# LittleDang/2DLIW-SLAM

Hardware: AMD Instinct MI355X
Metric: sliding-window solves/sec (30 KF, 2k scan pts) (higher is better)
Workload: dtype f64; 1 GPU; C2 synthetic: 49152 windows/GPU x (n=30 frames, L=2000 laser_factor blocks, 29 IMU + 29 wheel, 1800 ground); step = init-topology LM solve (cap 50 iters) + marginalization per window; windows_per_gpu=49152, frames=30, laser_blocks=2000, parallelism=windows replicated over 1 GPU(s), no data-path collective, distinct_windows_per_gpu=64

## Files before the change

### 2dliw-slam_amd/csrc/k_linearize.hip

```cpp
#include <type_traits>
#include <cstring>
#include "liw_kernels.hpp"

namespace liw {

__device__ __forceinline__ void frame_tf_record(const DevParams& P, const double* pose6, int dir, double* o) {
    V3<LJ> p = cast_v3<LJ>(pose6);
    V3<LJ> th(LJ(pose6[3], dir == 0 ? 1.0 : 0.0), LJ(pose6[4], dir == 1 ? 1.0 : 0.0), LJ(pose6[5], dir == 2 ? 1.0 : 0.0));
    Iso<LJ> Twl = mul(make_tf(p, th), cast_iso<LJ>(P.Ril, P.til));
    const LJ tt[2] = {Twl.t.x, Twl.t.y};
    if (dir == 3) {
        for (int r = 0; r < 2; ++r) { for (int c = 0; c < 3; ++c) o[r * 3 + c] = Twl.R(r, c).v; o[6 + r] = tt[r].v; }
    } else {
        for (int r = 0; r < 2; ++r) { for (int c = 0; c < 3; ++c) o[8 + 6 * dir + r * 3 + c] = Twl.R(r, c).d; o[26 + 2 * dir + r] = tt[r].d; }
    }
}
template <int V, int BIT>
__device__ __forceinline__ void bfly_step(double* v, int lane) {
    if constexpr (V > 1) {
        const bool up = (lane & BIT) != 0;
#pragma unroll
        for (int j = 0; j < V / 2; ++j) {
            const double send = up ? v[j] : v[j + V / 2];
            const double keep = up ? v[j + V / 2] : v[j];
// ... 636 lines not shown
    for (int e = 0; e < PGS; ++e) {
        int r = 0, c = e;
        while (c >= 7 - r) { c -= 7 - r; ++r; }
        t.e[e] = (r << 8) | (c + r);
    }
    return t;
}
__constant__ GroundRcTab c_ground_rc = make_ground_rc();
template <bool COSTCOPY>
__device__ __forceinline__ void ground_frames(const LinArgs& A, const DevParams& P, int wave, double* lds, const int* const act) {
    const int lane = threadIdx.x & 63, sub = lane >> 1, g = lane & 1;
    const int n = A.n;
    const long total = (long)(act ? act[0] : A.B) * n, gf = (long)wave * GROUND_PER_WAVE + sub;
    bool on = gf < total;
    const int wi = on ? (int)(gf / n) : 0;
    const int b = act ? act[1 + wi] : wi;
    if (on && !act) on = window_live(A, b);
    double* Y = lds + sub * 16;
    const size_t fi = on ? (size_t)b * n + (size_t)(gf % n) : 0;
    if (on) {
        const double* s_ = A.x + fi * 15;
        J3 res[2];
        {
            V3<J3> q;
            q.x = seed<3>(s_[3], 0, g == 1); q.y = seed<3>(s_[4], 1, g == 1); q.z = seed<3>(s_[5], 2, g == 1);
            const M3<J3> R = exp_so3(q);
            const J3 pz = seed<3>(s_[2], 2, g == 0);
            res[0] = (R(2, 0) * P.tiw[0] + R(2, 1) * P.tiw[1] + R(2, 2) * P.tiw[2] + pz) * P.ground_p_info;
            const J3 zx = R(0, 0) * P.Riw[2] + R(0, 1) * P.Riw[5] + R(0, 2) * P.Riw[8];
            const J3 zy = R(1, 0) * P.Riw[2] + R(1, 1) * P.Riw[5] + R(1, 2) * P.Riw[8];
            res[1] = dasin(dsqrt(zy * zy + zx * zx)) * P.ground_q_info;
        }
#pragma unroll
        for (int e = 0; e < 3; ++e) { Y[3 * g + e] = res[0].d[e]; Y[7 + 3 * g + e] = res[1].d[e]; }
        if (g == 0) { Y[6] = res[0].v; Y[13] = res[1].v; }
        if (g == 0 && A.dbg_ground_res) { A.dbg_ground_res[fi * 2] = res[0].v; A.dbg_ground_res[fi * 2 + 1] = res[1].v; }
        if (A.dbg_ground_jac)
            for (int e = 0; e < 3; ++e) { A.dbg_ground_jac[(fi * 2) * 6 + 3 * g + e] = res[0].d[e]; A.dbg_ground_jac[(fi * 2 + 1) * 6 + 3 * g + e] = res[1].d[e]; }
    }
    int* meta = reinterpret_cast<int*>(lds + GROUND_PER_WAVE * 16);
    if (g == 0) { meta[sub] = on ? (A.lm ? (A.candidate ? 1 - A.lm[b].cur : A.lm[b].cur) : 0) : -1; meta[32 + sub] = (int)fi; meta[64 + sub] = (int)cs_index(n, b, CS_GROUND, (int)(gf % n)); }
    lds_sync();
    {
        const long gf0 = (long)wave * GROUND_PER_WAVE;
        const int nfr = (int)min((long)GROUND_PER_WAVE, total - gf0);
        const double mult = (double)n;
        constexpr int LPF = PGS / 2;
        const int j = lane / LPF, pr = lane - j * LPF;
        const bool all_on = __builtin_amdgcn_ballot_w64(lane < nfr && meta[lane & 31] < 0) == 0;
        if (j < 4) {
            const int rc0 = c_ground_rc.e[2 * pr], rc1 = c_ground_rc.e[2 * pr + 1];
            const int r0 = rc0 >> 8, c0 = rc0 & 255, r1 = rc1 >> 8, c1 = rc1 & 255;
            auto frame = [&](int q) {
                const double* Yq = lds + q * 16;
                double2 v;
                v.x = mult * __builtin_fma(Yq[7 + r0], Yq[7 + c0], Yq[r0] * Yq[c0]);
                v.y = mult * __builtin_fma(Yq[7 + r1], Yq[7 + c1], Yq[r1] * Yq[c1]);
                return v;
            };
            auto put = [&](int sel, int fq, const double2& v) { *reinterpret_cast<double2*>(&(sel ? A.PG[1] : A.PG[0])[(size_t)fq * PGS + 2 * pr]) = v; };
            int q = j;
            if (all_on)
                for (; q + 4 < nfr; q += 8) {
                    const int sa = meta[q], fa = meta[32 + q], sb = meta[q + 4], fb = meta[36 + q];
                    const double2 va = frame(q), vb = frame(q + 4);
                    put(sa, fa, va); put(sb, fb, vb);
                }
            for (; q < nfr; q += 4) {
                const int sel = meta[q], fq = meta[32 + q];
                const double2 v = frame(q);
                if (sel >= 0) put(sel, fq, v);
            }
        }
        if (COSTCOPY && A.CS[0] && lane < nfr && meta[lane & 31] >= 0) {
            const double* Yq = lds + lane * 16;
            (meta[lane] ? A.CS[1] : A.CS[0])[meta[64 + lane]] = mult * __builtin_fma(Yq[13], Yq[13], Yq[6] * Yq[6]);
        }
    }
}

constexpr int WG_PER_WAVE = 31, WG_REC = 68;
constexpr int WG_LDS = WG_PER_WAVE * WG_REC + 96;
__device__ __forceinline__ LJN<4> ext4(const J3& a) { LJN<4> r; r.v = a.v; r.d[0] = a.d[0]; r.d[1] = a.d[1]; r.d[2] = a.d[2]; r.d[3] = 0.0; return r; }
template <bool COSTCOPY>
__device__ __forceinline__ void wheel_ground2_blocks(const LinArgs& A, const DevParams& P, int wave, double* lds, const int* const act) {
    typedef LJN<4> J4;
    typedef LJN<6> J6;
    const int lane = threadIdx.x & 63, blk = lane >> 1, f = lane & 1;
    const int n = A.n, nb = n - 1;
    const long total = (long)(act ? act[0] : A.B) * nb, gb = (long)wave * A.small_per_wave + blk;
    bool on = blk < A.small_per_wave && blk < WG_PER_WAVE && gb < total;
    const int wi = on ? (int)(gb / nb) : 0, k = on ? (int)(gb % nb) : 0;
    const int b = act ? act[1 + wi] : wi;
    if (on && !act) on = window_live(A, b);
    double* Y = lds + (blk < WG_PER_WAVE ? blk : 0) * WG_REC;
    const size_t fk = on ? (size_t)b * nb + k : 0, fi0 = on ? (size_t)b * n + k : 0;
    if (on) {
        const double* si_ = A.x + fi0 * 15;
        const double* sj_ = si_ + 15;
        const double* T12 = A.wheel_T + fk * 12;
        const double* sq9 = A.wheel_sqrtP + fk * 9;
        const V3<double> thi = cast_v3<double>(si_ + 3), thj = cast_v3<double>(sj_ + 3);
        V3<J3> arg;
        arg.x = seed<3>(f ? thj.x : thi.x, 0, true); arg.y = seed<3>(f ? thj.y : thi.y, 1, true); arg.z = seed<3>(f ? thj.z : thi.z, 2, true);
        const M3<J3> Md = exp_so3(arg);
        M3<double> Ri, Rj;
        {
            const int l0 = lane - f;
#pragma unroll
            for (int q = 0; q < 9; ++q) {
                const double mv = Md.m[q].v;
                Ri.m[q] = __shfl(mv, l0, 64);
                Rj.m[q] = __shfl(mv, l0 + 1, 64);
            }
        }
        {
            const double pz = f ? sj_[2] : si_[2];
            const J3 r0 = (Md(2, 0) * P.tiw[0] + Md(2, 1) * P.tiw[1] + Md(2, 2) * P.tiw[2] + J3(pz)) * P.ground_p_info;
            const J4 zx = ext4(Md(0, 0)) * P.Riw[2] + ext4(Md(0, 1)) * P.Riw[5] + ext4(Md(0, 2)) * P.Riw[8];
            const J4 zy = ext4(Md(1, 0)) * P.Riw[2] + ext4(Md(1, 1)) * P.Riw[5] + ext4(Md(1, 2)) * P.Riw[8];
            const J4 r1 = dasin(dsqrt(zy * zy + zx * zx)) * P.ground_q_info;
            double* Yg = Y + (f ? 39 : 53);
            Yg[0] = 0.0; Yg[1] = 0.0; Yg[2] = P.ground_p_info;
#pragma unroll
            for (int e = 0; e < 3; ++e) { Yg[3 + e] = r0.d[e]; Yg[7 + e] = r1.d[3]; Yg[10 + e] = r1.d[e]; }
            Yg[6] = r0.v; Yg[13] = r1.v;
            const size_t fi = fi0 + f;
            if ((f || k == 0) && A.dbg_ground_res) { A.dbg_ground_res[fi * 2] = r0.v; A.dbg_ground_res[fi * 2 + 1] = r1.v; }
            if ((f || k == 0) && A.dbg_ground_jac)
                for (int e = 0; e < 6; ++e) { A.dbg_ground_jac[(fi * 2) * 6 + e] = Yg[e]; A.dbg_ground_jac[(fi * 2 + 1) * 6 + e] = Yg[7 + e]; }
        }
        __builtin_amdgcn_sched_barrier(0);
        const M3<double> Riw = cast_m3<double>(P.Riw);
        const V3<double> tiw(P.tiw[0], P.tiw[1], P.tiw[2]);
        const M3<double> Rwi = mul(Ri, Riw);
        const M3<double> Am = transpose(Rwi);
        const M3<double> RjRiw = mul(Rj, Riw);
        const V3<double> Rjt = mul(Rj, tiw);
        const V3<double> w(Rjt.x + sj_[0] - si_[0], Rjt.y + sj_[1] - si_[1], Rjt.z + sj_[2] - si_[2]);
        const M3<double> Rrel = mul(Am, RjRiw);
        const V3<double> trel = mul(Am, w) - mulT(Riw, tiw);
        M3<J4> E;
        V3<J6> p;
#pragma unroll
        for (int q = 0; q < 9; ++q) E.m[q] = J4(Rrel.m[q]);
        p.x = J6(trel.x); p.y = J6(trel.y); p.z = J6(trel.z);
        p.x.d[3] = 1.0; p.y.d[4] = 1.0; p.z.d[5] = 1.0;
        {
            const M3<double> RiwT = transpose(Riw);
            M3<double> Lm, Rm;
#pragma unroll
            for (int q = 0; q < 9; ++q) { Lm.m[q] = f == 0 ? RiwT.m[q] : Am.m[q]; Rm.m[q] = f == 0 ? RjRiw.m[q] : Riw.m[q]; }
            const V3<double> wv(f == 0 ? w.x : tiw.x, f == 0 ? w.y : tiw.y, f == 0 ? w.z : tiw.z);
#pragma unroll
            for (int e = 0; e < 3; ++e) {
                M3<double> X;
#pragma unroll
                for (int r = 0; r < 3; ++r)
#pragma unroll
                    for (int c = 0; c < 3; ++c) X(r, c) = f == 0 ? Md(c, r).d[e] : Md(r, c).d[e];
                const M3<double> LX = mul(Lm, X);
                const M3<double> dR = mul(LX, Rm);
                const V3<double> dt = mul(LX, wv);
#pragma unroll
                for (int q = 0; q < 9; ++q) E.m[q].d[e] = dR.m[q];
                p.x.d[e] = dt.x; p.y.d[e] = dt.y; p.z.d[e] = dt.z;
            }
        }
        __builtin_amdgcn_sched_barrier(0);
        const V3<J4> q = log_SO3(E);
        const V3<double> oq = log_SO3(cast_m3<double>(T12));
        const double opx = T12[9], opy = T12[10];
        const double o_len = sqrt(opx * opx + opy * opy);
        const J6 len = dsqrt(p.x * p.x + p.y * p.y);
        J6 res0, res1, angle(0.0);
        if (o_len > 0.0001 && len.v > 0.0001) {
            const double odx = opx / o_len, ody = opy / o_len;
            const J6 dx = p.x / len, dy = p.y / len;
            const J6 cz = dy * odx - dx * ody;
            angle = dasin(dsqrt(cz * cz));
        } else {
            angle = len;
        }
        if (len.v < 0.0001 || o_len < 0.0001) res0 = len * sq9[0];
        else res0 = (J6(o_len) - len) * sq9[0];
        res1 = angle * sq9[4];
        const J4 nq = norm(q);
        const double noq = sqrt(oq.x * oq.x + oq.y * oq.y + oq.z * oq.z);
        J4 res2;
        if (nq.v < 0.001 || noq < 0.001) res2 = nq * sq9[8];
        else res2 = (J4(noq) - nq) * sq9[8];
#pragma unroll
        for (int e = 0; e < 3; ++e) {
            const int col = f ? 9 + e : 3 + e;
            Y[col] = res0.d[e]; Y[13 + col] = res1.d[e]; Y[26 + col] = res2.d[e];
        }
        if (f == 0) {
            const double Dp[3][3] = {{res0.d[3], res0.d[4], res0.d[5]}, {res1.d[3], res1.d[4], res1.d[5]}, {res2.d[3], res2.d[3], res2.d[3]}};
#pragma unroll
            for (int r = 0; r < 3; ++r) {
#pragma unroll
                for (int c = 0; c < 3; ++c) {
                    const double v = Dp[r][0] * Rwi.m[c * 3] + Dp[r][1] * Rwi.m[c * 3 + 1] + Dp[r][2] * Rwi.m[c * 3 + 2];
                    Y[r * 13 + 6 + c] = v;
                    Y[r * 13 + c] = -v;
                }
            }
            Y[12] = res0.v; Y[25] = res1.v; Y[38] = res2.v;
        }
    }
    lds_sync();
    if (on && f == 0 && A.dbg_wheel_res)
        for (int r = 0; r < 3; ++r) A.dbg_wheel_res[fk * 3 + r] = Y[r * 13 + 12];
    if (on && A.dbg_wheel_jac)
        for (int e = f; e < 36; e += 2) A.dbg_wheel_jac[fk * 36 + e] = Y[(e / 12) * 13 + e % 12];
    int* meta = reinterpret_cast<int*>(lds + WG_PER_WAVE * WG_REC);
    if (f == 0 && blk < WG_PER_WAVE) {
        meta[blk] = on ? (A.lm ? (A.candidate ? 1 - A.lm[b].cur : A.lm[b].cur) : 0) : -1;
        meta[32 + blk] = (int)fk;
        meta[64 + blk] = (int)cs_index(n, b, CS_WHEEL, k);
        meta[96 + blk] = (int)fi0;
        meta[128 + blk] = (int)cs_index(n, b, CS_GROUND, k);
        meta[160 + blk] = k;
    }
    lds_sync();
    const long gb0 = (long)wave * A.small_per_wave;
    const int nblk = (int)min((long)min(A.small_per_wave, WG_PER_WAVE), total - gb0);
    const int ml = lane < WG_PER_WAVE ? lane : 0;
    const int selv = meta[ml], fkv = meta[32 + ml], csv = meta[64 + ml], fiv = meta[96 + ml], cgv = meta[128 + ml], kv = meta[160 + ml];
    const bool all_on = __builtin_amdgcn_ballot_w64(lane < nblk && selv < 0) == 0;
    if (lane < PWS / 2) {
        const int rc0 = c_wheel_rc.e[2 * lane], rc1 = c_wheel_rc.e[2 * lane + 1];
        const int r0 = rc0 >> 8, c0 = rc0 & 255;
        const int r1 = rc1 >= 0 ? rc1 >> 8 : 0, c1 = rc1 >= 0 ? rc1 & 255 : 0;
        auto block = [&](int q) {
            const double* Yq = lds + q * WG_REC;
            double2 v;
            v.x = __builtin_fma(Yq[26 + r0], Yq[26 + c0], __builtin_fma(Yq[r0], Yq[c0], Yq[13 + r0] * Yq[13 + c0]));
            const double w1 = __builtin_fma(Yq[26 + r1], Yq[26 + c1], __builtin_fma(Yq[r1], Yq[c1], Yq[13 + r1] * Yq[13 + c1]));
            v.y = rc1 >= 0 ? w1 : 0.0;
            return v;
        };
        auto put = [&](int q, const double2& v) {
            const int sel = __builtin_amdgcn_readlane(selv, q);
            *reinterpret_cast<double2*>(&(sel ? A.PW[1] : A.PW[0])[(size_t)__builtin_amdgcn_readlane(fkv, q) * PWS + 2 * lane]) = v;
        };
        int q = 0;
        if (all_on)
            for (; q + 3 <= nblk; q += 3) {
                const double2 va = block(q), vb = block(q + 1), vc = block(q + 2);
                put(q, va); put(q + 1, vb); put(q + 2, vc);
            }
        for (; q < nblk; ++q) {
            const double2 v = block(q);
            if (__builtin_amdgcn_readlane(selv, q) >= 0) put(q, v);
        }
    }
    {
        const double mult = (double)n;
        constexpr int LPF = PGS / 2;
        const int j = lane / LPF, pr = lane - j * LPF;
        const bool any_k0 = __builtin_amdgcn_ballot_w64(lane < nblk && kv == 0) != 0;
        if (j < 4) {
            const int rc0 = c_ground_rc.e[2 * pr], rc1 = c_ground_rc.e[2 * pr + 1];
            const int r0 = rc0 >> 8, c0 = rc0 & 255, r1 = rc1 >> 8, c1 = rc1 & 255;
            for (int pass = 0; pass < (any_k0 ? 2 : 1); ++pass) {
                const int yo = pass ? 53 : 39;
                for (int q = j; q < nblk; q += 4) {
                    const int sel = meta[q], fq = meta[96 + q] + (pass ? 0 : 1), kq = meta[160 + q];
                    const double* Yq = lds + q * WG_REC + yo;
                    double2 v;
                    v.x = mult * __builtin_fma(Yq[7 + r0], Yq[7 + c0], Yq[r0] * Yq[c0]);
                    v.y = mult * __builtin_fma(Yq[7 + r1], Yq[7 + c1], Yq[r1] * Yq[c1]);
                    if (sel >= 0 && (pass == 0 || kq == 0))
                        *reinterpret_cast<double2*>(&(sel ? A.PG[1] : A.PG[0])[(size_t)fq * PGS + 2 * pr]) = v;
                }
            }
        }
        if (COSTCOPY && A.CS[0] && lane < nblk && selv >= 0) {
            const double* Yq = lds + lane * WG_REC;
            double* CSb = selv ? A.CS[1] : A.CS[0];
            CSb[csv] = __builtin_fma(Yq[38], Yq[38], __builtin_fma(Yq[12], Yq[12], Yq[25] * Yq[25]));
            CSb[cgv + 1] = mult * __builtin_fma(Yq[39 + 13], Yq[39 + 13], Yq[39 + 6] * Yq[39 + 6]);
            if (kv == 0) CSb[cgv] = mult * __builtin_fma(Yq[53 + 13], Yq[53 + 13], Yq[53 + 6] * Yq[53 + 6]);
        }
        (void)fiv;
    }
}

__host__ __device__ inline int imu_wave_count(int B, int n, int per_wave) { return n > 1 ? (int)(((long)B * (n - 1) + per_wave - 1) / per_wave) : 0; }
__host__ __device__ inline int wheel_wave_count(int B, int n, int per_wave) { return imu_wave_count(B, n, per_wave); }
__host__ __device__ inline int ground_wave_count(int B, int n) { return (int)(((long)B * n + GROUND_PER_WAVE - 1) / GROUND_PER_WAVE); }
template <int ND, bool COSTCOPY>
__device__ __forceinline__ void small_role(const LinArgs& A, const DevParams& P, int vblock, double* lds, const int* const act) {
    const int nw = wheel_wave_count(A.B, A.n, A.small_per_wave);
    if (vblock < nw) wheel_blocks<ND, COSTCOPY>(A, P, vblock, lds, act);
    else ground_frames<COSTCOPY>(A, P, vblock - nw, lds, act);
}
constexpr int SMALL_LDS = WHEEL_PER_WAVE * 64 + 32 + 16 + 64;
__global__ __launch_bounds__(64, 2) void k_lin_imu(LinArgs A, DevParams P) {
    __shared__ double lds[IMU_PER_WAVE * IMU_REC];
    const int* const act = usable_active_list(A.active, A.B);
    if (A.imu_pk && *A.imu_pk_bad == 0) imu_blocks<3, true>(A, P, (int)blockIdx.x, lds, act);
    else imu_blocks<3>(A, P, (int)blockIdx.x, lds, act);
}
__global__ __launch_bounds__(64, 2) void k_lin_imu_chain(LinArgs A, DevParams P) {
    __shared__ __attribute__((aligned(16))) double lds[IMU_PER_WAVE * IMU_REC + IMU_STAGE + IMU_SBUF];
    const int* const act = usable_active_list(A.active, A.B);
    if (A.imu_pk && *A.imu_pk_bad == 0) imu_blocks<3, true, true>(A, P, (int)blockIdx.x, lds, act);
    else imu_blocks<3, false, true>(A, P, (int)blockIdx.x, lds, act);
}
__global__ __launch_bounds__(64, 2) void k_lin_imu_chain_multi(LinArgs A, DevParams P) {
    __shared__ __attribute__((aligned(16))) double lds[IMU_PER_WAVE * IMU_REC + IMU_STAGE + IMU_SBUF];
    const int* const act = usable_active_list(A.active, A.B);
    if (A.imu_pk && *A.imu_pk_bad == 0) imu_blocks<3, true, true, true>(A, P, (int)blockIdx.x, lds, act);
    else imu_blocks<3, false, true, true>(A, P, (int)blockIdx.x, lds, act);
}
__global__ void k_imu_pack(long blocks, const double* X, const double* J, const double* S, const double* Dt, double* pk, int* bad) {
    const long t = (long)blockIdx.x * blockDim.x + threadIdx.x;
    if (t >= blocks * 256) return;
    const long fk = t >> 8;
    const int e = (int)(t & 255);
    if (e < IMU_PK) {
        double v = 0.0;
        if (e < 15) v = X[fk * 15 + e];
        else if (e == IPK_DT) v = Dt[fk];
        else if (e < IPK_S) { const int q = e - IPK_J; v = J[fk * 225 + (q / 6) * 15 + 9 + q % 6]; }
        else if (e < IPK_S + 120) {
            int r = 0, q = e - IPK_S;
            while (q >= 15 - r) { q -= 15 - r; ++r; }
            v = S[fk * 225 + r * 15 + r + q];
        }
        pk[fk * IMU_PK + e] = v;
    }
    if (e < 225 && e % 15 < e / 15 && S[fk * 225 + e] != 0.0) atomicOr(bad, 1);
}
__global__ void k_laser_z_scan(long Ltot, const double* pts, int* flag) {
    const long t = (long)blockIdx.x * blockDim.x + threadIdx.x;
    bool nz = false;
    for (long j = t; j < Ltot; j += (long)gridDim.x * blockDim.x)
        nz = nz || pts[2 * Ltot + j] != 0.0 || pts[5 * Ltot + j] != 0.0 || pts[8 * Ltot + j] != 0.0 || pts[11 * Ltot + j] != 0.0;
    if (__any(nz) && (threadIdx.x & 63) == 0) atomicOr(flag, 1);
}
void launch_laser_z_scan(long Ltot, const double* laser_pts, int* flag, hipStream_t s) {
    (void)hipMemsetAsync(flag, 0, sizeof(int), s);
    if (Ltot <= 0) return;
    const long blocks = (Ltot + 1023) / 1024;
    hipLaunchKernelGGL(k_laser_z_scan, dim3((unsigned)(blocks < 4096 ? blocks : 4096)), dim3(256), 0, s, Ltot, laser_pts, flag);
}
void launch_imu_pack(int B, int n, const double* imu_X, const double* imu_J, const double* imu_sqrtP, const double* imu_Dt, double* pk, int* bad, hipStream_t s) {
    (void)hipMemsetAsync(bad, 0, sizeof(int), s);
    const long blocks = (long)B * (n - 1);
    if (blocks <= 0) return;
    hipLaunchKernelGGL(k_imu_pack, dim3((unsigned)blocks), dim3(256), 0, s, blocks, imu_X, imu_J, imu_sqrtP, imu_Dt, pk, bad);
}
constexpr int SMALL_OCC = 2;
__global__ __launch_bounds__(64, SMALL_OCC) void k_lin_small(LinArgs A, DevParams P) {
    __shared__ double lds[WG_LDS > SMALL_LDS ? WG_LDS : SMALL_LDS];
    static_assert(sizeof(double) * (WG_LDS > SMALL_LDS ? WG_LDS : SMALL_LDS) * 4 * SMALL_OCC <= 160 * 1024, "LDS of the waves of a CU");
    const int* const act = usable_active_list(A.active, A.B);
    if (A.n > 1) wheel_ground2_blocks<true>(A, P, (int)blockIdx.x, lds, act);
    else ground_frames<true>(A, P, (int)blockIdx.x, lds, act);
}
__global__ void k_lm_reset(int B, LmState* lm, int max_iters) {
    const int b = blockIdx.x * blockDim.x + threadIdx.x;
    if (b < B) lm_reset(lm[b], max_iters);
}
template <bool BOTH>
__global__ __launch_bounds__(64, 2) void k_lin_all(LinArgs A, DevParams P, int G, int n_laser, int n_imu, int n_roles) {
    __shared__ double lds[IMU_PER_WAVE * IMU_REC];
    const int v = (int)blockIdx.x;
    if (v >= n_roles) {
        for (int b = threadIdx.x; b < A.B; b += 64) lm_reset(A.reset_lm[b], A.reset_iters);
        return;
    }
#ifdef LIW_CLK
    if ((threadIdx.x & 63) == 0 && v < 40) g_clk_lin[400 + 2 * v] = clock64();
#endif
    if (v < n_laser) laser_wave_local<BOTH>(A, P, G, v);
    else if (A.small_nd == 1) {
        if (v < n_laser + n_imu) imu_blocks<1>(A, P, v - n_laser, lds, nullptr); else small_role<1, false>(A, P, v - n_laser - n_imu, lds, nullptr);
    } else {
        if (v < n_laser + n_imu) imu_blocks<3>(A, P, v - n_laser, lds, nullptr); else small_role<3, false>(A, P, v - n_laser - n_imu, lds, nullptr);
    }
#ifdef LIW_CLK
    asm volatile("s_waitcnt vmcnt(0) lgkmcnt(0)" ::: "memory");
    if ((threadIdx.x & 63) == 0 && v < 40) g_clk_lin[401 + 2 * v] = clock64();
#endif
}

constexpr int COMPACT_MAX = 1 << 20;
__host__ __device__ inline size_t compact_pub_offset(int B) { return (sizeof(int) * ((size_t)B + 3) + 7) & ~(size_t)7; }
__host__ __device__ inline size_t compact_list_bytes(int B) { return compact_pub_offset(B) + 8 * (((size_t)B + 255) / 256); }
__global__ __launch_bounds__(256) void k_compact_active(int B, const LmState* lm, int* active) {
    unsigned long long* pub = reinterpret_cast<unsigned long long*>(reinterpret_cast<char*>(active) + compact_pub_offset(B));
    int* ticket = active + B + 1;
    int* status = active + B + 2;
    __shared__ int wcnt[4];
    __shared__ int part[4];
    const int t = threadIdx.x, lane = t & 63, wv = t >> 6, blk = (int)blockIdx.x, nblk = (int)gridDim.x;
    const int b0 = blk * 256 + t;
    const bool live = b0 < B && !lm[b0].done;
    const unsigned long long m = __ballot(live);
    const int before = __popcll(m & ((1ull << lane) - 1ull));
    if (lane == 0) wcnt[wv] = __popcll(m);
    __syncthreads();
    const int bc = wcnt[0] + wcnt[1] + wcnt[2] + wcnt[3];
    if (t == 0) __hip_atomic_store(pub + blk, ((unsigned long long)bc << 1) | 1ull, __ATOMIC_RELEASE, __HIP_MEMORY_SCOPE_AGENT);
    int sum = 0;
    for (int j = t; j < blk; j += 256) {
        unsigned long long v = 0;
        for (long polls = 0; polls < (1l << 24); ++polls) {
            v = __hip_atomic_load(pub + j, __ATOMIC_ACQUIRE, __HIP_MEMORY_SCOPE_AGENT);
            if (v & 1ull) break;
            __builtin_amdgcn_s_sleep(2);
        }
        if (!(v & 1ull)) atomicOr(status, 2);
        sum += (int)(v >> 1);
    }
    for (int o = 32; o > 0; o >>= 1) sum += __shfl_xor(sum, o, 64);
    if (lane == 0) part[wv] = sum;
    __syncthreads();
    const int offset = part[0] + part[1] + part[2] + part[3];
    int wbase = 0;
    for (int q = 0; q < wv; ++q) wbase += wcnt[q];
    if (live) active[1 + offset + wbase + before] = b0;
    if (blk == nblk - 1 && t == 0) { active[0] = offset + bc; atomicOr(status, 1); }
    __syncthreads();
    if (t == 0 && __hip_atomic_fetch_add(ticket, 1, __ATOMIC_ACQ_REL, __HIP_MEMORY_SCOPE_AGENT) == nblk - 1) {
        for (int j = 0; j < nblk; ++j) __hip_atomic_store(pub + j, 0ull, __ATOMIC_RELAXED, __HIP_MEMORY_SCOPE_AGENT);
        __hip_atomic_store(ticket, 0, __ATOMIC_RELEASE, __HIP_MEMORY_SCOPE_AGENT);
    }
}

__global__ void k_group_offsets(int B, int n, const int* laser_off, const int* laser_frame, int* group_off) {
    const int t = blockIdx.x * blockDim.x + threadIdx.x;
    if (t >= B * (n + 1)) return;
    const int b = t / (n + 1), i = t % (n + 1);
    int lo = laser_off[b], hi = laser_off[b + 1];
    while (lo < hi) {
        const int mid = (lo + hi) >> 1;
        if (laser_frame[mid] < i) lo = mid + 1; else hi = mid;
    }
    group_off[t] = lo;
}

size_t compact_list_bytes_host(int B) { return compact_list_bytes(B); }
bool lin_builds_active_list(int B, int eval_small) {
    static const bool no_compact = getenv("LIW_NO_COMPACT") != nullptr;
    return eval_small && B >= 512 && B <= COMPACT_MAX && !no_compact;
}
void launch_linearize(const LinArgs& A_, const DevParams& P, hipStream_t s, const LinFork* fk, bool defer_join) {
    LinArgs A = A_;
    const int n = A.n, B = A.B;
    A.small_nd = 3;
    {
        const long blocks = (long)B * (n > 1 ? n - 1 : 0);
        int pw = WHEEL_PER_WAVE;
        while (pw > 3 && (blocks + pw - 1) / pw < 512) pw = (pw + 1) / 2;
        const bool nd3 = getenv("LIW_SMALL_ND3") != nullptr;
        if (A.eval_small && !nd3 && !A.pi_frame && A.role_mask == 0 && (long)B * n + 2 * blocks + ground_wave_count(B, n) <= 256) { pw = 1; A.small_nd = 1; }
        A.small_per_wave = pw;
        A.imu_per_wave = pw < IMU_PER_WAVE ? pw : IMU_PER_WAVE;
    }
    int G = 1;
    if (A.mode != LIW_MODE_TRACK) while (G < LASER_GMAX && (long)B * ((n + 2 * G - 1) / (2 * G)) >= 4096) G *= 2;
    const int laser_waves = B * ((n + G - 1) / G);
    const int imu_waves = A.eval_small ? imu_wave_count(B, n, A.imu_per_wave) : 0;
    const int small_waves = A.eval_small ? wheel_wave_count(B, n, A.small_per_wave) + ground_wave_count(B, n) : 0;
    const bool have_list = A.lm && A.active && lin_builds_active_list(B, A.eval_small);
    const bool compact = have_list && (A.role_mask == 0 || (A.role_mask & 8));
    if (!have_list) A.active = nullptr;
    if (!A.pi_frame && A.role_mask == 0 && laser_waves + imu_waves + small_waves <= 256) {
        const int roles = laser_waves + imu_waves + small_waves;
        const unsigned tot = (unsigned)(roles + (A.reset_lm ? 1 : 0));
        if (A.mode == LIW_MODE_INIT) hipLaunchKernelGGL(k_lin_all<true>, dim3(tot), dim3(64), 0, s, A, P, G, laser_waves, imu_waves, roles);
        else hipLaunchKernelGGL(k_lin_all<false>, dim3(tot), dim3(64), 0, s, A, P, G, laser_waves, imu_waves, roles);
        return;
    }
    if (A.reset_lm) hipLaunchKernelGGL(k_lm_reset, dim3((B + 63) / 64), dim3(64), 0, s, B, A.reset_lm, A.reset_iters);
    const bool fork = fk && fk->side[0] && A.eval_small;
    if (compact) hipLaunchKernelGGL(k_compact_active, dim3((unsigned)((B + 255) / 256)), dim3(256), 0, s, B, A.lm, A.active);
    if (fork) {
        hipEventRecord(fk->ev_fork, s);
        hipStreamWaitEvent(fk->side[0], fk->ev_fork, 0);
        hipStreamWaitEvent(fk->side[1], fk->ev_fork, 0);
    }
    hipStream_t s_imu = fork ? fk->side[0] : s, s_small = fork ? fk->side[1] : s;
    const int rm = A.role_mask ? A.role_mask : 7;
    auto role_laser = [&]() {
        if (!(rm & 1)) return;
        if (A.laser_pk) launch_lin_laser_slab(A, P, s);
        else if (A.mode == LIW_MODE_INIT) hipLaunchKernelGGL(k_lin_laser<true>, dim3((unsigned)laser_waves), dim3(64), 0, s, A, P, G);
        else hipLaunchKernelGGL(k_lin_laser<false>, dim3((unsigned)laser_waves), dim3(64), 0, s, A, P, G);
    };
    auto role_imu = [&]() {
        const bool no_multi = getenv("LIW_NO_IMU_MULTI") != nullptr;
        if (imu_waves && (rm & 2) && A.pi_frame && imu_chain_windows(n - 1) > 1 && !no_multi) {
            const int wpw = imu_chain_windows(n - 1);
            hipLaunchKernelGGL(k_lin_imu_chain_multi, dim3((unsigned)((B + wpw - 1) / wpw)), dim3(64), 0, s_imu, A, P);
        } else if (imu_waves && (rm & 2) && A.pi_frame) hipLaunchKernelGGL(k_lin_imu_chain, dim3((unsigned)(B * imu_chain_parts(n - 1))), dim3(64), 0, s_imu, A, P);
        else if (imu_waves && (rm & 2)) hipLaunchKernelGGL(k_lin_imu, dim3((unsigned)imu_waves), dim3(64), 0, s_imu, A, P);
    };
    auto role_small = [&]() {
        if (!(small_waves && (rm & 4))) return;
        if (A.small_per_wave == WHEEL_PER_WAVE) A.small_per_wave = WG_PER_WAVE;
        const int waves = n > 1 ? wheel_wave_count(B, n, A.small_per_wave) : ground_wave_count(B, n);
        hipLaunchKernelGGL(k_lin_small, dim3((unsigned)waves), dim3(64), 0, s_small, A, P);
    };
    static const char* order_env = getenv("LIW_LIN_ORDER");
    const char* order = (order_env && strlen(order_env) == 3) ? order_env : "lis";
    for (int k = 0; k < 3; ++k) {
        if (order[k] == 'l') role_laser();
        else if (order[k] == 'i') role_imu();
        else if (order[k] == 's') role_small();
    }
    if (fork) {
        hipEventRecord(fk->ev_join[0], fk->side[0]);
        hipEventRecord(fk->ev_join[1], fk->side[1]);
        if (!defer_join) {
            hipStreamWaitEvent(s, fk->ev_join[0], 0);
            hipStreamWaitEvent(s, fk->ev_join[1], 0);
        }
    }
}
void launch_linearize_join(hipStream_t s, const LinFork* fk) {
    if (!fk || !fk->side[0]) return;
    hipStreamWaitEvent(s, fk->ev_join[0], 0);
    hipStreamWaitEvent(s, fk->ev_join[1], 0);
}

__global__ void k_exchange_pack(int groups, int n, int np, int compact, LaserPackTable tb, const double* PL0, const double* PL1, int candidate, const LmState* lm, double* buf) {
    const int t = blockIdx.x * blockDim.x + threadIdx.x;
    if (t >= groups * np) return;
    const int grp = t / np, p = t % np;
    const bool dead = lm && lm[grp / n].done;
    const int sel = lm ? (candidate ? 1 - lm[grp / n].cur : lm[grp / n].cur) : 0;
    const double* PL = sel ? PL1 : PL0;
    double v;
    if (compact) v = PL[(size_t)grp * LPC + p];
    else { v = PL[(size_t)grp * LP + tb.slot[p]]; v = tb.neg[p] ? -v : v; }
    buf[t] = dead ? 0.0 : v;
}
template <bool BOTH>
__global__ void k_exchange_unpack(int groups, int n, int np, int compact, int world, size_t stride, const double* buf, double* PL0, double* PL1, double* CS0, double* CS1, int candidate, const LmState* lm, int sysload) {
    const int t = blockIdx.x * blockDim.x + threadIdx.x;
    const int lps = laser_stride(compact);
    if (t >= groups * lps) return;
    const int grp = t / lps, s = t % lps;
    const int sel = lm ? (candidate ? 1 - lm[grp / n].cur : lm[grp / n].cur) : 0;
    double* PL = sel ? PL1 : PL0;
    const int code = compact ? (s < np ? s : -1) : laser_slot_code<BOTH>(s);
    double v = 0.0;
    if (code >= 0) {
        const double* src = buf + (size_t)grp * np + (code & 63);
        for (int r = 0; r < world; ++r)
            v += sysload ? __hip_atomic_load(src + (size_t)r * stride, __ATOMIC_RELAXED, __HIP_MEMORY_SCOPE_SYSTEM) : src[(size_t)r * stride];
        if (code & 64) v = -v;
    }
    PL[t] = v;
    if (s == (compact ? np - 1 : 120) && CS0) (sel ? CS1 : CS0)[cs_index(n, grp / n, CS_LASER, grp % n)] = v;
}
template <bool BOTH>
__global__ void k_laser_expand(int groups, int compact, const double* PL, double* out) {
    const size_t t = (size_t)blockIdx.x * blockDim.x + threadIdx.x;
    if (t >= (size_t)groups * LP) return;
    out[t] = laser_slot<BOTH>(PL + (t / LP) * laser_stride(compact), (int)(t % LP), compact);
}
void launch_laser_expand(int B, int n, bool both, int compact, const double* PL, double* out, hipStream_t s) {
    const int groups = B * n;
    const unsigned blocks = (unsigned)(((size_t)groups * LP + 255) / 256);
    if (both) hipLaunchKernelGGL(k_laser_expand<true>, dim3(blocks), dim3(256), 0, s, groups, compact, PL, out);
    else hipLaunchKernelGGL(k_laser_expand<false>, dim3(blocks), dim3(256), 0, s, groups, compact, PL, out);
}
__global__ void k_count_active(int B, const LmState* lm, double* out) {
    __shared__ int cnt;
    if (threadIdx.x == 0) cnt = 0;
    __syncthreads();
    int c = 0;
    for (int b = threadIdx.x; b < B; b += blockDim.x) c += lm[b].done ? 0 : 1;
    atomicAdd(&cnt, c);
    __syncthreads();
    if (threadIdx.x == 0) out[0] = (double)cnt;
}
void launch_exchange_pack(int B, int n, bool both, int compact, const double* PL0, const double* PL1, int candidate, const LmState* lm, double* buf, hipStream_t s) {
    const int np = both ? 45 : 21, groups = B * n;
    LaserPackTable tb{};
    for (int p = 0; p < np; ++p) tb.slot[p] = -1;
    for (int sl = 0; sl < LP; ++sl) {
        const int code = both ? laser_slot_code<true>(sl) : laser_slot_code<false>(sl);
// ... 52 lines not shown
```

### 2dliw-slam_amd/csrc/k_lm.hip

```cpp
#include "liw_kernels.hpp"
#include "k_lm_common.hpp"

namespace liw {

typedef double d4 __attribute__((ext_vector_type(4)));
#ifdef LIW_CLK
__device__ long long g_clk[8192];
__device__ long long g_span[3 * 16384];
#ifndef LIW_CLK_IT
#define LIW_CLK_IT 3
#endif
#define STAMP(id) do { if (b == 0 && lane == 0 && iteration_dbg == LIW_CLK_IT) g_clk[(id)] = clock64(); } while (0)
#define STAMPE(id) do { if (b == 0 && lane == 0 && iteration == LIW_CLK_IT) g_clk[(id)] = clock64(); } while (0)
#define STAMPM(id) do { if (b == 0 && lane == 0) g_clk[(id)] = clock64(); } while (0)
#define JSTAMP(id) do { if (t == 0 && blockIdx.x == 0 && sweep == 1 && rnd == 3) g_clk[(id)] = clock64(); } while (0)
#define JSTAMPV(id, v) do { double w_ = (v); asm volatile("" : "+v"(w_)); if (t == 0 && blockIdx.x == 0 && sweep == 1 && rnd == 3) g_clk[(id)] = clock64(); } while (0)
#define SPAN(k) do { if (lane == 0 && iteration_dbg == LIW_CLK_IT && b < 16384) { g_span[3 * b + (k)] = clock64(); \
                     if ((k) == 0) g_span[3 * b + 2] = __builtin_amdgcn_s_getreg((4 << 0) | (0 << 6) | (31 << 11)); } } while (0)
#else
#define STAMP(id) do { } while (0)
#define STAMPE(id) do { } while (0)
#define STAMPM(id) do { } while (0)
#define JSTAMP(id) do { } while (0)
#define JSTAMPV(id, v) do { } while (0)
#define SPAN(k) do { } while (0)
#endif


struct AsmCtx {
    int n, mode, fast, b, buf;
    int pif;
    int plc;
    const double* PL; const double* PI; const double* PW; const double* PG;
    const double* x;
    const double* pJ; const double* pX; bool prior_on;
};
__device__ __forceinline__ AsmCtx asm_ctx(const WsView& w, int n, int mode, int fast, int b, const double* prior_J, const double* prior_X, bool prior_on) {
    AsmCtx c;
    c.pif = w.pi_frame; c.plc = w.pl_compact; c.n = n; c.mode = mode; c.fast = fast; c.b = b;
    c.pJ = prior_J + (size_t)b * 225; c.pX = prior_X + (size_t)b * 15; c.prior_on = prior_on;
    return c;
}
__device__ __forceinline__ void bind(AsmCtx& c, const WsView& w, int buf, const double* x) {
    c.buf = buf; c.PL = w.PL[buf]; c.PI = w.PI[buf]; c.PW = w.PW[buf]; c.PG = w.PG[buf]; c.x = x;
}

__device__ __forceinline__ void copy_states(double* dst, const double* src, int n, int lane) {
    for (int e = lane; e < n * 15; e += 64) dst[e] = src[e];
}
__device__ __forceinline__ double free_norm(const double* x, int mode, int fast, int n, int lane) {
    double s = 0.0;
    for (int e = lane; e < n * 15; e += 64) if (!var_is_const(mode, fast, n, e / 15, e % 15)) s += x[e] * x[e];
    return sqrt(wave_sum(s));
}
__device__ __forceinline__ void history_put(const StepArgs& a, int rec, int b, const double* x, int lane) {
    if (a.w.history && rec < a.w.history_records)
        for (int e = lane; e < a.n * 15; e += 64) a.w.history[((size_t)rec * a.B + b) * a.n * 15 + e] = x[e];
}
__device__ __forceinline__ void lm_store_exit(LmState& st, int term, double radius, double dec, double x_cost, double x_norm, int reuse, int cur) {
    st.done = 1; st.termination = term; st.radius = radius; st.decrease_factor = dec; st.x_cost = x_cost; st.x_norm = x_norm;
    st.reuse_diagonal = reuse; st.cur = cur; st.have_candidate = 0;
}

__device__ __forceinline__ double prior_r(const AsmCtx& c, int k) {
    const double* xs = c.x + (size_t)(c.n - 2) * 15;
    double s = 0.0;
    for (int j = 0; j < 15; ++j) s += c.pJ[k * 15 + j] * (xs[j] - c.pX[j]);
    return s;
}

__device__ __forceinline__ double pl_slot(const AsmCtx& c, const double* rec, int s) { return laser_slot(rec, s, c.plc, c.mode == LIW_MODE_INIT); }

struct FrameExtra { double sc_i, sc_m, dg_i, x_i; };

constexpr int MS = 41;
template <int LAYOUT> struct Tiles {
    double* D; double* O; double* R; double* g;
    __device__ __forceinline__ double& d(int r, int c) const { return LAYOUT ? D[r * MS + c] : D[r * 16 + c]; }
    __device__ __forceinline__ double& o(int r, int c) const { return LAYOUT ? D[c * MS + 16 + r] : O[r * 16 + c]; }
    __device__ __forceinline__ double& rr(int r, int c) const { return LAYOUT ? D[c * MS + 32 + r] : R[r * 16 + c]; }
    __device__ __forceinline__ double& gg(int r) const { return LAYOUT ? D[r * MS + 40] : g[r]; }
};

struct AsmRegs {
    double v5[4], v6[4], v7[4];
    double t1, t2, t3, t4, t8, t9, t10;
    double g1, g2, g3, g4, g5, g6;
    double xq, sc_i, sc_m, dg_i;
    double e1[2], e2;
};
struct PriorRegs { double pj[4], pdx; };
__device__ __forceinline__ PriorRegs prior_issue(const AsmCtx& c, int lane) {
    PriorRegs P;
#pragma unroll
    for (int q = 0; q < 4; ++q) {
        const int e = lane + 64 * q, r = e >> 4, cc = e & 15;
        P.pj[q] = (r < 15 && cc < 15) ? c.pJ[r * 15 + cc] : 0.0;
    }
    const int v = lane < 15 ? lane : 0;
    P.pdx = c.x[(size_t)(c.n - 2) * 15 + v] - c.pX[v];
    return P;
}
constexpr int ASM_TMP = 16;

__device__ __forceinline__ AsmRegs asm_issue(const AsmCtx& c, int i, const double* scl, const double* dgl, int lane = threadIdx.x & 63, int dir = -1) {
    const int n = c.n;
    const bool up = dir > 0;
    const int LPS = laser_stride(c.plc);
    const double* PLb = c.PL + (size_t)c.b * n * LPS;
    const bool pif = c.pif != 0;
    const bool hasm = i >= 1, hasp = i <= n - 2;
    const double* PIb = c.PI + (size_t)c.b * (pif ? (size_t)n * PIFS : (size_t)(n - 1) * PIS);
    const double* PWb = c.PW + (size_t)c.b * (n - 1) * PWS;
    const double* PGb = c.PG + (size_t)c.b * n * PGS;
    const double* PIm = pif ? PIb + (size_t)i * PIFS : PIb + (size_t)(hasm ? i - 1 : 0) * PIS;
    const double* PIp = pif ? PIb + (size_t)(hasp ? i + 1 : i) * PIFS : PIb + (size_t)(hasp ? i : 0) * PIS;
    const int oJJ = pif ? PIF_D : PI_JJ, oIJ = pif ? PIF_IJ : PI_IJ;
    const double* PWm = PWb + (size_t)(hasm ? i - 1 : 0) * PWS;
    const double* PWp = PWb + (size_t)(hasp ? i : 0) * PWS;
    const double* PLi = PLb + (size_t)i * LPS;
    const double* PL1 = PLb + (size_t)(n > 1 ? 1 : 0) * LPS;
    const double* PGi = PGb + (size_t)i * PGS;
    AsmRegs R;
#pragma unroll
    for (int q = 0; q < 4; ++q) {
        const int e = lane + 64 * q, r = e >> 4, cc = e & 15;
        const bool valid = r < 15 && cc < 15;
        const int rs = valid ? r : 0, cs = valid ? cc : 0;
        const int tq = pi_tri(rs, cs);
        R.v5[q] = PIm[(unsigned)(oJJ + tq)];
        R.v6[q] = pif ? 0.0 : PIp[(unsigned)(PI_II + tq)];
        R.v7[q] = up ? PIp[(unsigned)(oIJ + cs * 15 + rs)] : PIm[(unsigned)(oIJ + rs * 15 + cs)];
    }
    {
        const bool pl = lane < 36;
        const int r = pl ? lane / 6 : 0, cc = pl ? lane % 6 : 0;
        R.t1 = pl_slot(c, PLi, 36 + r * 6 + cc);
        R.t2 = PWm[(unsigned)PW_JJ(r, cc)];
        R.t3 = PWp[(unsigned)PW_II(r, cc)];
        R.t4 = PGi[(unsigned)PG_H(r, cc)];
        R.t8 = up ? PWp[(unsigned)PW_IJ(cc, r)] : PWm[(unsigned)PW_IJ(r, cc)];
        R.e2 = up ? PWm[(unsigned)PW_IJ(r, cc)] : 0.0;
        R.t9 = pl_slot(c, PL1, 72 + r * 6 + cc);
        R.t10 = pl_slot(c, PLi, 72 + r * 6 + cc);
    }
    {
        const int r = lane < 15 ? lane : 0, r6 = r < 6 ? r : 0;
        R.g1 = pl_slot(c, PLi, 114 + r6);
        R.g2 = PWm[(unsigned)PW_G(6 + r6)];
        R.g3 = PWp[(unsigned)PW_G(r6)];
        R.g4 = PGi[(unsigned)PG_G(r6)];
        R.g5 = PIm[(unsigned)((pif ? PIF_GJ : PI_G + 15) + r)];
        R.g6 = pif ? PIm[(unsigned)(PIF_GI + r)] : PIp[(unsigned)(PI_G + r)];
    }
    const int nbf = up ? (hasp ? i + 1 : i) : (hasm ? i - 1 : i);
    {
        int idx = i * 15 + (lane < 15 ? lane : 0);
        if (lane >= 16 && lane < 19) idx = nbf * 15 + 3 + (lane - 16);
        if (lane >= 20 && lane < 23) idx = 3 + (lane - 20);
        R.xq = c.x[(unsigned)idx];
        const int v = lane < 15 ? lane : 0;
        R.sc_i = scl ? scl[(unsigned)(i * 15 + v)] : 1.0;
        R.sc_m = scl ? scl[(unsigned)(nbf * 15 + v)] : 1.0;
        R.dg_i = dgl ? dgl[(unsigned)(i * 15 + v)] : 0.0;
    }
#pragma unroll
    for (int q = 0; q < 2; ++q) {
        const int e = lane + 64 * q;
        R.e1[q] = up ? PIm[(unsigned)(oIJ + (e < 90 ? e : 0))] : 0.0;
    }
    return R;
}

__device__ __forceinline__ d4 xty16(const double* X, const double* Y);
template <int LAYOUT>
__device__ void asm_commit(const AsmCtx& c, int i, const AsmRegs& R, const Tiles<LAYOUT>& T_, double* tmp, FrameExtra* ex = nullptr,
                           int lane = threadIdx.x & 63, int dir = -1, const PriorRegs* pr = nullptr) {
    const int n = c.n;
    const int LPS = laser_stride(c.plc);
    const double* PLb = c.PL + (size_t)c.b * n * LPS;
    const bool hasm = i >= 1, hasp = i <= n - 2;
    const bool up = dir > 0, hasnb = up ? hasp : hasm;
    const int nbf = up ? (hasp ? i + 1 : i) : (hasm ? i - 1 : i);
    const bool arrow1 = up && i == 1;
    const bool prior_here = c.prior_on && i == n - 2;
    d4 jtj = {0.0, 0.0, 0.0, 0.0};
    double gprior = 0.0;
    if (prior_here) {
        double* Jt = T_.D;
        double* dxp = LAYOUT ? T_.D + 256 : T_.O;
        const PriorRegs P_ = pr ? *pr : prior_issue(c, lane);
#pragma unroll
        for (int q = 0; q < 4; ++q) Jt[lane + 64 * q] = P_.pj[q];
        if (lane < 16) dxp[lane] = lane < 15 ? P_.pdx : 0.0;
        lds_sync();
        if (lane < 15) {
            double sp = 0.0;
#pragma unroll
            for (int j = 0; j < 15; ++j) sp += Jt[lane * 16 + j] * dxp[j];
            tmp[lane] = sp;
        }
        jtj = xty16(Jt, Jt);
        lds_sync();
        if (lane < 15) {
#pragma unroll
            for (int k = 0; k < 15; ++k) gprior += Jt[k * 16 + lane] * tmp[k];
        }
        lds_sync();
    }
    double dI[4], oI[4];
#pragma unroll
    for (int q = 0; q < 4; ++q) {
        const int e = lane + 64 * q, r = e >> 4, cc = e & 15;
        const bool valid = r < 15 && cc < 15;
        dI[q] = ((valid && (c.pif ? n > 1 : hasm)) ? R.v5[q] : 0.0) + ((valid && hasp && !c.pif) ? R.v6[q] : 0.0);
        oI[q] = (valid && hasnb) ? R.v7[q] : 0.0;
    }
    double dP = 0.0, oP = 0.0, rP = 0.0;
    {
        const bool pl = lane < 36;
        const int r = pl ? lane / 6 : 0, cc = pl ? lane % 6 : 0;
        dP = R.t1 + (hasm ? R.t2 : 0.0) + (hasp ? R.t3 : 0.0) + R.t4;
        if (i == 0 && c.mode == LIW_MODE_INIT) {
            double s0 = 0.0, s1 = 0.0, s2 = 0.0, s3 = 0.0;
            int j = 0;
            for (; j + 4 <= n; j += 4) {
                s0 += pl_slot(c, PLb + (size_t)j * LPS, r * 6 + cc); s1 += pl_slot(c, PLb + (size_t)(j + 1) * LPS, r * 6 + cc);
                s2 += pl_slot(c, PLb + (size_t)(j + 2) * LPS, r * 6 + cc); s3 += pl_slot(c, PLb + (size_t)(j + 3) * LPS, r * 6 + cc);
            }
            for (; j < n; ++j) s0 += pl_slot(c, PLb + (size_t)j * LPS, r * 6 + cc);
            dP += (s0 + s1) + (s2 + s3);
        }
        oP = hasnb ? R.t8 + ((!up && i == 1) ? R.t9 : 0.0) : 0.0;
        rP = (i >= 2 || arrow1) ? R.t10 + (arrow1 ? R.e2 : 0.0) : 0.0;
        if (!pl) { dP = 0.0; oP = 0.0; rP = 0.0; }
    }
    double gg = 0.0;
    {
        const int r = lane < 15 ? lane : 0;
        if (r < 6) {
            gg = R.g1 + (hasm ? R.g2 : 0.0) + (hasp ? R.g3 : 0.0) + R.g4;
            if (i == 0 && c.mode == LIW_MODE_INIT) {
                double s0 = 0.0, s1 = 0.0, s2 = 0.0, s3 = 0.0;
                int j = 0;
                for (; j + 4 <= n; j += 4) {
                    s0 += pl_slot(c, PLb + (size_t)j * LPS, 108 + r); s1 += pl_slot(c, PLb + (size_t)(j + 1) * LPS, 108 + r);
                    s2 += pl_slot(c, PLb + (size_t)(j + 2) * LPS, 108 + r); s3 += pl_slot(c, PLb + (size_t)(j + 3) * LPS, 108 + r);
                }
                for (; j < n; ++j) s0 += pl_slot(c, PLb + (size_t)j * LPS, 108 + r);
                gg += (s0 + s1) + (s2 + s3);
            }
        }
        gg += (hasm ? R.g5 : 0.0) + (hasp ? R.g6 : 0.0);
    }
    const double xq = R.xq;
    if (ex) { ex->sc_i = R.sc_i; ex->sc_m = R.sc_m; ex->dg_i = R.dg_i; ex->x_i = xq; }
#pragma unroll
    for (int q = 0; q < 4; ++q) {
        const int e = lane + 64 * q;
        const int r = e >> 4, cc = e & 15;
        const bool valid = r < 15 && cc < 15;
        double d = dI[q];
        if (prior_here && valid) d += jtj[q];
        if (LAYOUT == 0) { T_.D[e] = valid ? d : 0.0; T_.O[e] = valid ? oI[q] : 0.0; T_.R[e] = 0.0; }
        else if (valid) { T_.d(r, cc) = d; T_.o(r, cc) = oI[q]; if (r < 6) T_.rr(r, cc) = 0.0; }
    }
    if (lane < 16) {
        double g = lane < 15 ? gg : 0.0;
        if (prior_here && lane < 15) g += gprior;
        if (LAYOUT == 0) T_.g[lane] = g; else if (lane < 15) T_.gg(lane) = g;
    }
    lds_sync();
    if (lane < 36) {
        const int r = lane / 6, cc = lane % 6;
        T_.d(r, cc) += dP; T_.o(r, cc) += oP; T_.rr(r, cc) = rP;
    }
    lds_sync();
    if (arrow1) {
#pragma unroll
        for (int q = 0; q < 2; ++q) {
            const int e = lane + 64 * q;
            if (e < 90) T_.rr(e / 15, e % 15) += R.e1[q];
        }
        lds_sync();
    }
    if (c.mode == LIW_MODE_MARG) return;
    double Pi[9], Pm[9], P0[9];
    const double qa0 = rdlane(xq, 3), qa1 = rdlane(xq, 4), qa2 = rdlane(xq, 5);
    const double qb0 = rdlane(xq, 16), qb1 = rdlane(xq, 17), qb2 = rdlane(xq, 18);
    const double qc0 = rdlane(xq, 20), qc1 = rdlane(xq, 21), qc2 = rdlane(xq, 22);
    const double pi2 = kPi * kPi;
    bool li = qa0 * qa0 + qa1 * qa1 + qa2 * qa2 > pi2;
    bool lm = hasnb && qb0 * qb0 + qb1 * qb1 + qb2 * qb2 > pi2;
    bool l0 = (i >= 2 || arrow1) && qc0 * qc0 + qc1 * qc1 + qc2 * qc2 > pi2;
    if (li || lm || l0) {
        li = so3_plus_jac(c.x + (size_t)i * 15 + 3, Pi);
        lm = hasnb && so3_plus_jac(c.x + (size_t)nbf * 15 + 3, Pm);
        l0 = (i >= 2 || arrow1) && so3_plus_jac(c.x + 3, P0);
        if (lane == 0) {
            auto at = [&](int kind, int r, int cc) -> double& { return kind == 0 ? T_.d(r, cc) : (kind == 1 ? T_.o(r, cc) : T_.rr(r, cc)); };
            auto right = [&](int kind, int nrows, const double* P) {
                for (int r = 0; r < nrows; ++r) {
                    double t[3];
                    for (int k = 0; k < 3; ++k) t[k] = at(kind, r, 3) * P[k] + at(kind, r, 4) * P[3 + k] + at(kind, r, 5) * P[6 + k];
                    for (int k = 0; k < 3; ++k) at(kind, r, 3 + k) = t[k];
                }
            };
            auto left = [&](int kind, const double* P) {
                for (int cc = 0; cc < 15; ++cc) {
                    double t[3];
                    for (int k = 0; k < 3; ++k) t[k] = P[k] * at(kind, 3, cc) + P[3 + k] * at(kind, 4, cc) + P[6 + k] * at(kind, 5, cc);
                    for (int k = 0; k < 3; ++k) at(kind, 3 + k, cc) = t[k];
                }
            };
            if (li) {
                right(0, 15, Pi); left(0, Pi); right(1, 15, Pi); right(2, 6, Pi);
                double t[3];
                for (int k = 0; k < 3; ++k) t[k] = Pi[k] * T_.gg(3) + Pi[3 + k] * T_.gg(4) + Pi[6 + k] * T_.gg(5);
                for (int k = 0; k < 3; ++k) T_.gg(3 + k) = t[k];
            }
            if (lm) left(1, Pm);
            if (l0) left(2, P0);
        }
        lds_sync();
    }
    if (c.mode == LIW_MODE_TRACK) {
        for (int e = lane; e < 256; e += 64) {
            const int r = e >> 4, cc = e & 15;
            if (r < 15 && cc < 15) {
                const bool cr = var_is_const(c.mode, c.fast, n, i, r), ccn = var_is_const(c.mode, c.fast, n, i, cc);
                if (cr || ccn) T_.d(r, cc) = 0.0;
                if ((hasnb && var_is_const(c.mode, c.fast, n, nbf, r)) || ccn) T_.o(r, cc) = 0.0;
                if (arrow1 && r < 6 && (var_is_const(c.mode, c.fast, n, 0, r) || ccn)) T_.rr(r, cc) = 0.0;
            }
        }
        if (lane < 15 && var_is_const(c.mode, c.fast, n, i, lane)) T_.gg(lane) = 0.0;
        lds_sync();
    }
}

template <int LAYOUT>
__device__ void assemble_frame(const AsmCtx& c, int i, const Tiles<LAYOUT>& T_, double* tmp,
                               const double* scl = nullptr, const double* dgl = nullptr, FrameExtra* ex = nullptr) {
    const AsmRegs R = asm_issue(c, i, scl, dgl);
    __builtin_amdgcn_sched_barrier(0);
    asm_commit<LAYOUT>(c, i, R, T_, tmp, ex);
}

__device__ double window_cost(const AsmCtx& c, double* gchk = nullptr) {
    const int lane = threadIdx.x & 63;
    const int n = c.n;
    const int LPS = laser_stride(c.plc);
    const double* PLb = c.PL + (size_t)c.b * n * LPS;
    const bool pif = c.pif != 0;
    const double* PIb = c.PI + (size_t)c.b * (pif ? (size_t)n * PIFS : (size_t)(n - 1) * PIS);
    const double* PWb = c.PW + (size_t)c.b * (n - 1) * PWS;
    const double* PGb = c.PG + (size_t)c.b * n * PGS;
    const bool track = c.mode == LIW_MODE_TRACK;
    double s = 0.0, gs = 0.0;
    for (int i = lane; i < n; i += 64) {
        const bool gon = !(track && i < n - 1);
        if (gon) s += pl_slot(c, PLb + (size_t)i * LPS, 120);
        if (gon) s += PGb[(size_t)i * PGS + PG_C];
        if (gchk) {
            if (gon) {
#pragma unroll
                for (int k = 0; k < 12; ++k) gs += pl_slot(c, PLb + (size_t)i * LPS, 108 + k);
            }
            if (gon) {
#pragma unroll
                for (int k = 0; k < 6; ++k) gs += PGb[(size_t)i * PGS + PG_G(k)];
            }
        }
    }
    for (int k = lane; k < n - 1; k += 64) {
        s += pif ? PIb[(size_t)(k + 1) * PIFS + PIF_C] : PIb[(size_t)k * PIS + PI_C];
        const bool won = !(track && k < n - 2);
        if (won) s += PWb[(size_t)k * PWS + PW_C];
        if (gchk) {
#pragma unroll
            for (int e = 0; e < 30; ++e)
                gs += pif ? (e < 15 ? PIb[(size_t)k * PIFS + PIF_GI + e] : PIb[(size_t)(k + 1) * PIFS + PIF_GJ + e - 15]) : PIb[(size_t)k * PIS + PI_G + e];
            if (won) {
#pragma unroll
                for (int e = 0; e < 12; ++e) gs += PWb[(size_t)k * PWS + PW_G(e)];
            }
        }
    }
    if (c.prior_on && lane < 15) { const double r = prior_r(c, lane); s += r * r; }
    if (gchk) *gchk = wave_sum(gs);
    return 0.5 * wave_sum(s);
}

__device__ __forceinline__ d4 xty16(const double* X, const double* Y) {
    const int lane = threadIdx.x & 63;
    d4 acc = {0.0, 0.0, 0.0, 0.0};
#pragma unroll
    for (int c = 0; c < 4; ++c) {
        const int k = (lane >> 4) + 4 * c;
        acc = __builtin_amdgcn_mfma_f64_16x16x4f64(X[k * 16 + (lane & 15)], Y[k * 16 + (lane & 15)], acc, 0, 0, 0);
    }
    return acc;
}

template <int XS, int YS>
__device__ __forceinline__ d4 xty15(const double* X, const double* Y, const double* Z) {
    const int lane = threadIdx.x & 63, m = lane & 15;
    d4 acc = {0.0, 0.0, 0.0, 0.0};
#pragma unroll
    for (int c = 0; c < 4; ++c) {
        const int k = (lane >> 4) + 4 * c;
        const double* xr = X + k * XS;
        const double* yr = Y + k * YS;
        if (c == 3) { const bool z = (lane >> 4) == 3; xr = z ? Z : xr; yr = z ? Z : yr; }
        acc = __builtin_amdgcn_mfma_f64_16x16x4f64(xr[m], yr[m], acc, 0, 0, 0);
    }
    return acc;
}

struct LdsTiles {
    double D[256], O[256], R[256], W[256], Wa[256], CD[256], CR[256];
    double g[16], Cg[16], y0[16], yprev[16], tmp[ASM_TMP], D0acc[36], g0acc[8], sci[16], scm[16], sc0[16], dgi[16];
};
struct LdsStep {
    double M[720], C[15 * MS], Z[16];
    double tmp[ASM_TMP], D0acc[36], g0acc[8];
};
constexpr int LW = 0, LLI = 240, LWA = 480;
struct LdsDense2 {
    LdsStep S;
    double D1[256], O1[256], R1[256], D0[256], O0[256], R0[256], g1[16], g0[16];
};
__device__ __forceinline__ LdsStep& step_lds(LdsStep& T) { return T; }
__device__ __forceinline__ LdsStep& step_lds(LdsDense2& T) { return T.S; }

template <int NP = 15>
__device__ __forceinline__ bool fused_chol_solve(double (&a)[15]) {
    bool ok = true;
#pragma unroll
    for (int k = 0; k < NP; ++k) {
        const double piv = rdlane(a[k], k);
        if (k == NP - 1 && (!(piv > 0.0) || !isfinite(piv))) ok = false;
        const double inv = fast_rsqrt(piv);
        const double wk = a[k] * inv;
        a[k] = wk;
#pragma unroll
        for (int r = k + 1; r < 15; ++r) a[r] -= rdlane(wk, r) * wk;
    }
    return ok;
}

__device__ __forceinline__ bool fused_chol_solve30(double (&a)[30], unsigned inert) {
    bool ok = true;
#pragma unroll
    for (int k = 0; k < 30; ++k) {
        if (k < 15 && ((inert >> k) & 1u)) continue;
        const double piv = rdlane(a[k], k);
        if (k == 29 && (!(piv > 0.0) || !isfinite(piv))) ok = false;
        const double inv = fast_rsqrt(piv);
        const double wk = a[k] * inv;
        a[k] = wk;
#pragma unroll
        for (int r = k + 1; r < 30; ++r) a[r] -= rdlane(wk, r) * wk;
    }
    return ok;
}

template <bool WAVE_ONLY = false>
__device__ double frame_diag(const AsmCtx& c, int i, LdsStep& T) {
    const int lane = threadIdx.x & 63, n = c.n;
    double Pq[9];
    if (so3_plus_jac(c.x + (size_t)i * 15 + 3, Pq)) {
        assemble_frame<1>(c, i, Tiles<1>{T.M, nullptr, nullptr, nullptr}, T.tmp);
        const double d = lane < 15 ? T.M[lane * MS + lane] : 0.0;
        lds_sync();
        return d;
    }
    if (lane >= 15) return 0.0;
    const int r = lane;
    const int LPS = laser_stride(c.plc);
    const double* PLb = c.PL + (size_t)c.b * n * LPS;
    const double* PIb = c.PI + (size_t)c.b * (c.pif ? (size_t)n * PIFS : (size_t)(n - 1) * PIS);
    const double* PWb = c.PW + (size_t)c.b * (n - 1) * PWS;
    const double* PGb = c.PG + (size_t)c.b * n * PGS;
    double d = 0.0;
    if (r < 6) {
        d += pl_slot(c, PLb + (size_t)i * LPS, 36 + r * 7);
        if (i == 0) for (int j = 0; j < n; ++j) d += pl_slot(c, PLb + (size_t)j * LPS, r * 7);
        if (i >= 1) d += PWb[(size_t)(i - 1) * PWS + PW_JJ(r, r)];
        if (i <= n - 2) d += PWb[(size_t)i * PWS + PW_II(r, r)];
        d += PGb[(size_t)i * PGS + PG_H(r, r)];
    }
    if (c.pif) { if (n > 1) d += PIb[(size_t)i * PIFS + PIF_D + pi_tri(r, r)]; }
    else {
        if (i >= 1) d += PIb[(size_t)(i - 1) * PIS + PI_JJ + pi_tri(r, r)];
        if (i <= n - 2) d += PIb[(size_t)i * PIS + PI_II + pi_tri(r, r)];
    }
    if (c.prior_on && i == n - 2) { double s = 0.0; for (int k = 0; k < 15; ++k) s += c.pJ[k * 15 + r] * c.pJ[k * 15 + r]; d += s; }
    return d;
}

struct BsRow { double row[22], gsv, xold, scv, dgv; };
__device__ __forceinline__ BsRow bs_fetch(const double* sws, const double* xw, const double* scl, const double* dgl, int i, int lane) {
    static_assert(REC_LD % 2 == 0 && SOLVE_WS % 2 == 0, "16-byte aligned record rows");
    const double* f = sws + (size_t)i * SOLVE_WS;
    const int r = lane < 15 ? lane : 0;
    const double2* f2 = reinterpret_cast<const double2*>(f + r * REC_LD);
    BsRow R;
#pragma unroll
    for (int k = 0; k < 11; ++k) { const double2 v = f2[k]; R.row[2 * k] = v.x; R.row[2 * k + 1] = v.y; }
    R.gsv = f[REC_GS + r]; R.xold = xw[(size_t)i * 15 + r]; R.scv = scl[i * 15 + r]; R.dgv = dgl[i * 15 + r];
    return R;
}
__device__ __forceinline__ void bs_emit(const StepArgs& a, int i, int lane, double t, const BsRow& R, double damp, double* xc, double& sn2, double& ytg, double& dsum) {
    const bool cst = lane < 15 && var_is_const(a.mode, a.fast_mode, a.n, i, lane);
    const double del = (lane < 15 && !cst) ? -t * R.scv : 0.0;
    const double qv[3] = {rdlane(R.xold, 3), rdlane(R.xold, 4), rdlane(R.xold, 5)};
    double dq[3] = {rdlane(del, 3), rdlane(del, 4), rdlane(del, 5)}, qn[3];
    so3_plus(qv, dq, qn);
    if (lane < 15) {
        double xnew = R.xold + del;
        if (lane >= 3 && lane < 6) xnew = var_is_const(a.mode, a.fast_mode, a.n, i, 3) ? R.xold : qn[lane - 3];
        xc[(size_t)i * 15 + lane] = xnew;
        if (!cst) {
            sn2 += (R.xold - xnew) * (R.xold - xnew);
            ytg += t * R.gsv;
            dsum += damp * t * t;
        }
    }
}

template <bool THROUGHPUT, bool DENSE2 = false, class LDS = LdsStep>
__device__ __forceinline__ void lm_step_body(const StepArgs& a, const int b, LDS& TL) {
    constexpr bool LIW_PF1 = !THROUGHPUT, LIW_PF2 = true;
    LdsStep& T = step_lds(TL);
    const int lane = threadIdx.x & 63;
    LmState& st = a.w.lm[b];
    if constexpr (DENSE2) {
        double pf_sink = 0.0;
        int done0 = st.done;
        const int n2 = a.n;
        const bool pr = a.mode == LIW_MODE_TRACK && !a.fast_mode;
        double v[14];
#pragma unroll
        for (int k = 0; k < 2; ++k) {
            v[4 * k + 0] = touch_lines(a.w.PL[k] + (size_t)b * n2 * laser_stride(a.w.pl_compact), sizeof(double) * n2 * laser_stride(a.w.pl_compact));
            v[4 * k + 1] = touch_lines(a.w.PI[k] + (size_t)b * (n2 - 1) * PIS, sizeof(double) * (n2 - 1) * PIS);
            v[4 * k + 2] = touch_lines(a.w.PW[k] + (size_t)b * (n2 - 1) * PWS, sizeof(double) * (n2 - 1) * PWS);
            v[4 * k + 3] = touch_lines(a.w.PG[k] + (size_t)b * n2 * PGS, sizeof(double) * n2 * PGS);
        }
        v[8] = touch_lines(a.x + (size_t)b * n2 * 15, sizeof(double) * n2 * 15);
        v[9] = touch_lines(a.w.x_cand + (size_t)b * n2 * 15, sizeof(double) * n2 * 15);
        v[10] = touch_lines(st.scale, sizeof(double) * n2 * 15);
        v[11] = touch_lines(st.diagonal, sizeof(double) * n2 * 15);
        {
            const double* const xb = a.x + (size_t)b * n2 * 15;
            const double* const PJ = a.prior_J; const double* const PX = a.prior_X;
            const bool pj = pr && PJ != nullptr, px = pr && PX != nullptr;
            const size_t qj = (size_t)(PJ + (size_t)b * 225), qx = (size_t)(PX + (size_t)b * 15), q0 = (size_t)xb;
            v[12] = touch_lines(reinterpret_cast<const void*>(pj ? qj : q0), pj ? sizeof(double) * 225 : sizeof(double) * 8);
            v[13] = touch_lines(reinterpret_cast<const void*>(px ? qx : q0), px ? sizeof(double) * 15 : sizeof(double) * 8);
        }
#pragma unroll
        for (int k = 0; k < 14; ++k) pf_sink += v[k];
        asm volatile("" : "+v"(pf_sink), "+v"(done0));
        if (done0) return;
    }
    if (st.done) return;
    if (a.only_slow) {
        const int taken = st.pad_;
        wave_mem_sync();
        if (taken) { if (lane == 0) st.pad_ = 0; return; }
    }
    const int n = a.n;
// ... 814 lines not shown
        } else if (a.mode == LIW_MODE_TRACK) {
            if (i == n - 1 && a.has_match[i]) a.match_pose[i * 12 + 6 + k] = a.x[(size_t)i * 15 + k];
        }
    }
    __syncthreads();
    int* hdr = reinterpret_cast<int*>(a.out);
    if (t == 0) { hdr[0] = a.lm[0].done; hdr[1] = a.marg_status ? a.marg_status[0] : 3; hdr[2] = 0; }
    if (t == 1) {
        const LmState& st = a.lm[0];
        liw_summary o;
        o.iterations = st.iteration; o.successful_steps = st.successful; o.termination = st.termination;
        o.initial_cost = st.initial_cost; o.final_cost = st.x_cost;
        *reinterpret_cast<liw_summary*>(a.out + 2) = o;
        a.info[0] = o;
    }
    double* o = a.out + LIW_RESULT_HDR;
    for (int e = t; e < n * 15; e += blockDim.x) o[e] = a.x[e];
    o += n * 15;
    for (int e = t; e < n * 12; e += blockDim.x) o[e] = a.match_pose[e];
    o += n * 12;
    if (a.marg) for (int e = t; e < 276; e += blockDim.x) o[e] = a.marg[e];
    __threadfence_system();
    __syncthreads();
    if (t == 0) { __threadfence_system(); __hip_atomic_store(hdr + 3, a.seq, __ATOMIC_RELEASE, __HIP_MEMORY_SCOPE_SYSTEM); }
}
__global__ void k_pack_result(PackArgs a) { pack_result_body(a); }

__global__ void k_lm_finish(StepArgs a) {
    const int t = blockIdx.x * blockDim.x + threadIdx.x;
    const int n = a.n;
    if (t >= a.B * n * 6) return;
    const int k = t % 6, i = (t / 6) % n, b = t / (6 * n);
    const double* xw = a.x + (size_t)b * n * 15;
    double* mp = a.match_pose + (size_t)b * n * 12;
    if (a.mode == LIW_MODE_INIT) {
        if (a.has_match[b * n + i]) { mp[i * 12 + k] = xw[k]; mp[i * 12 + 6 + k] = xw[(size_t)i * 15 + k]; }
    } else if (a.mode == LIW_MODE_TRACK) {
        if (i == n - 1 && a.has_match[b * n + i]) mp[i * 12 + 6 + k] = xw[(size_t)i * 15 + k];
    }
    if (i == 0 && k == 0) {
        const LmState& st = a.w.lm[b];
        liw_summary& o = a.w.info[b];
        o.iterations = st.iteration; o.successful_steps = st.successful; o.termination = st.termination;
        o.initial_cost = st.initial_cost; o.final_cost = st.x_cost;
    }
}

__global__ __launch_bounds__(64) void k_export_dense(ExportArgs a) {
    __shared__ LdsTiles T;
    const int b = blockIdx.x, lane = threadIdx.x & 63, n = a.n, N = 15 * n;
    AsmCtx c = asm_ctx(a.w, n, a.mode, a.fast_mode, b, a.prior_J, a.prior_X,
                       a.has_prior[b] && ((a.mode == LIW_MODE_TRACK && !a.fast_mode) || a.mode == LIW_MODE_MARG));
    bind(c, a.w, 0, a.x + (size_t)b * n * 15);
    c.buf = a.buf;
    double* H = a.H + (size_t)b * N * N;
    double* g = a.g + (size_t)b * N;
    for (size_t e = lane; e < (size_t)N * N; e += 64) H[e] = 0.0;
    __syncthreads();
    const double sgn = a.mode == LIW_MODE_MARG ? -1.0 : 1.0;
    for (int i = 0; i < n; ++i) {
        assemble_frame<0>(c, i, Tiles<0>{T.D, T.O, T.R, T.g}, T.tmp);
        for (int e = lane; e < 256; e += 64) {
            const int r = e >> 4, cc = e & 15;
            if (r < 15 && cc < 15) {
                H[(size_t)(i * 15 + r) * N + i * 15 + cc] = T.D[e];
                if (i >= 1) { H[(size_t)((i - 1) * 15 + r) * N + i * 15 + cc] = T.O[e]; H[(size_t)(i * 15 + cc) * N + (i - 1) * 15 + r] = T.O[e]; }
                if (i >= 2 && r < 6) { H[(size_t)r * N + i * 15 + cc] = T.R[e]; H[(size_t)(i * 15 + cc) * N + r] = T.R[e]; }
            }
        }
        if (lane < 15) g[i * 15 + lane] = sgn * T.g[lane];
        __syncthreads();
    }
    const double cst = window_cost(c);
    if (lane == 0) a.cost[b] = cst;
}

template <class TILES>
__device__ __forceinline__ bool marg_chain(const MargArgs& a, const int b, TILES& T) {
    const int lane = threadIdx.x & 63, n = a.n;
    AsmCtx c = asm_ctx(a.w, n, LIW_MODE_MARG, 0, b, a.prior_J, a.prior_X, a.has_prior[b] != 0);
    const int sel = a.use_cur ? __builtin_amdgcn_readfirstlane(a.w.lm[b].cur) : 0;
    c.buf = sel; c.x = a.x + (size_t)b * n * 15;
    c.PL = sel ? a.w.PL[1] : a.w.PL[0]; c.PI = sel ? a.w.PI[1] : a.w.PI[0]; c.PW = sel ? a.w.PW[1] : a.w.PW[0]; c.PG = sel ? a.w.PG[1] : a.w.PG[0];
    STAMPM(5000);
    for (int e = lane; e < 256; e += 64) { T.CD[e] = 0.0; T.W[e] = 0.0; }
    if (lane < 16) T.Cg[lane] = 0.0;
    lds_sync();
    bool ok = true;
    double* Dc = T.D; double* gc = T.g;
    double* Dn = T.Wa; double* gn = T.y0;
    assemble_frame<0>(c, 0, Tiles<0>{Dc, T.O, T.R, gc}, T.tmp);
    AsmRegs areg = asm_issue(c, n > 1 ? 1 : 0, nullptr, nullptr);
    for (int i = 0; i + 1 < n; ++i) {
        asm_commit<0>(c, i + 1, areg, Tiles<0>{Dn, T.O, T.R, gn}, T.tmp);
        __builtin_amdgcn_sched_barrier(0);
        if (i + 2 < n) areg = asm_issue(c, i + 2, nullptr, nullptr);
        __builtin_amdgcn_sched_barrier(0);
        double col[15];
        {
            const bool ml_ = lane < 15, ol_ = lane >= 16 && lane < 31, gl_ = lane == 40;
            const double* pA = ml_ ? Dc + lane : (ol_ ? T.O + (lane - 16) : (gl_ ? gc : T.R));
            const double* pB = ml_ ? T.CD + lane : (gl_ ? T.Cg : (ol_ ? T.Cg + 15 : T.R));
            const int st = gl_ ? 1 : 16, stB = ol_ ? 0 : st;
#pragma unroll
            for (int r = 0; r < 15; ++r) col[r] = pA[r * st] + pB[r * stB];
        }
        if (!fused_chol_solve(col)) { ok = false; break; }
        if ((lane >= 16 && lane < 31) || lane == 40) {
            double* const wc = T.W + (lane == 40 ? 15 : lane - 16);
#pragma unroll
            for (int r = 0; r < 15; ++r) wc[r * 16] = col[r];
        }
        lds_sync();
        const d4 p1 = xty16(T.W, T.W);
        lds_sync();
#pragma unroll
        for (int r = 0; r < 4; ++r) {
            const int row = (lane >> 4) + 4 * r, colx = lane & 15;
            if (row < 15 && colx < 15) T.CD[row * 16 + colx] = -p1[r];
            if (row < 15 && colx == 15) T.Cg[row] = -p1[r];
        }
        lds_sync();
        double* t1 = Dc; Dc = Dn; Dn = t1;
        double* t2 = gc; gc = gn; gn = t2;
    }
    {
        double dv[4], gv = 0.0;
#pragma unroll
        for (int q = 0; q < 4; ++q) {
            const int e = lane + 64 * q, r = e >> 4, cc = e & 15;
            dv[q] = (r < 15 && cc < 15) ? Dc[e] + T.CD[e] : 0.0;
        }
        if (lane < 15) gv = gc[lane] + T.Cg[lane];
        lds_sync();
#pragma unroll
        for (int q = 0; q < 4; ++q) T.D[lane + 64 * q] = dv[q];
        if (lane < 16) T.g[lane] = lane < 15 ? gv : 0.0;
        lds_sync();
    }
    if (a.status && lane == 0) a.status[b] = ok ? 0 : 1;
    if (!ok) return false;
    if (a.Delta_H) for (int e = lane; e < 225; e += 64) a.Delta_H[(size_t)b * 225 + e] = T.D[(e / 15) * 16 + e % 15];
    if (a.Delta_g && lane < 15) a.Delta_g[(size_t)b * 15 + lane] = -T.g[lane];
    return true;
}

__device__ __forceinline__ void jacobi_rotation(double d, double h, double& cs, double& sn) {
    const double qq = d * d + h * h;
    const double r = qq * fast_rsqrt(qq);
    const double u = fabs(d) + r;
    const double winv = fast_rsqrt(2.0 * r * u);
    cs = u * winv;
    sn = (d >= 0.0 ? h : -h) * winv;
}
template <class TILES>
__device__ __forceinline__ void jacobi15_wave(TILES& T, double* V, double* Am, double* rot) {
    const int lane = threadIdx.x & 63;
    for (int e = lane; e < 256; e += 64) {
        const int r = e >> 4, cc = e & 15;
        Am[e] = (r < 15 && cc < 15) ? 0.5 * (T.D[r * 16 + cc] + T.D[cc * 16 + r]) : 0.0;
        V[e] = r == cc ? 1.0 : 0.0;
    }
    lds_sync();
    for (int sweep = 0; sweep < 60; ++sweep) {
        double off = 0.0, dgn = 0.0;
        for (int e = lane; e < 225; e += 64) {
// ... 410 lines not shown
```

### 2dliw-slam_amd/csrc/k_lm_quad.hip

```cpp
#include <cstddef>
#include <cstdlib>
#include <type_traits>

#include "liw_kernels.hpp"
#include "k_lm_common.hpp"

namespace liw {

template <int B_, int E_, class F> __device__ __forceinline__ void sfor(F&& f) {
    if constexpr (B_ < E_) { f(std::integral_constant<int, B_>{}); sfor<B_ + 1, E_>(f); }
}
#define KI(K) (std::remove_reference_t<decltype(K)>::value)
template <int V> using KC = std::integral_constant<int, V>;
__device__ __forceinline__ double bits_and(double x, unsigned long long m) { return __longlong_as_double((long long)((unsigned long long)__double_as_longlong(x) & m)); }

template <int L> __device__ __forceinline__ double bc(double v) {
    double r;
    asm volatile("v_mov_b64_dpp %0, %1 row_newbcast:%2 row_mask:0xf bank_mask:0xf" : "=v"(r) : "v"(v), "n"(L));
    return r;
}
template <int L> __device__ __forceinline__ void fnma_bc(double& acc, double src, double mul) {
    asm volatile("v_fmac_f64_dpp %0, -%1, %2 row_newbcast:%3 row_mask:0xf bank_mask:0xf" : "+v"(acc) : "v"(src), "v"(mul), "n"(L));
}
template <int L> __device__ __forceinline__ double mul_bc(double src, double mul) {
    double r;
    asm volatile("v_mul_f64_dpp %0, %1, %2 row_newbcast:%3 row_mask:0xf bank_mask:0xf" : "=v"(r) : "v"(src), "v"(mul), "n"(L));
    return r;
}
__device__ __forceinline__ double mul_nop(double x, double y) {
    double r;
    asm volatile("v_mul_f64 %0, %1, %2\n s_nop 1" : "=v"(r) : "v"(x), "v"(y));
    return r;
}
__device__ __forceinline__ void dpp_fence() { asm volatile("s_nop 1"); }

__device__ __forceinline__ double row_max(double v) {
    v = fmax(v, dpp64<0xB1>(v, v)); v = fmax(v, dpp64<0x4E>(v, v)); v = fmax(v, dpp64<0x141>(v, v)); v = fmax(v, dpp64<0x140>(v, v));
    return v;
}

__device__ long long g_qclk[64];
__device__ int g_qclk_on[4];
#define QSTAMP(id) do { if (clk_on && i == clk_frame) { if (lane == 0) g_qclk[(id)] = clock64(); } } while (0)

constexpr int QTR = 4 * 15 * 6;
constexpr int K_A = 0, K_B = 6, K_C = 12, K_HA = 18, K_D = 24, K_CW = 39, K_GSH = 45, K_RL = 46, NRD = 52;
constexpr int QTAB = NRD * 16;
constexpr int QZB = 86;
constexpr int QPAD = 96;
constexpr int QTOT_1 = 4 * (PIFS + LPC + PWS + PGS) + QPAD + QTR + QZB + QTAB;
constexpr int quad_laser_slot(int kind, int r, int j) {
    return kind == 0 ? (j == 15 ? 114 + r : 36 + r * 6 + j) : kind == 1 ? (j == 15 ? 108 + r : r * 6 + j) : 72 + j * 6 + r;
}
template <bool BOTH> constexpr bool quad_sign_rows_ok() {
    for (int jj = 0; jj < 7; ++jj) {
        const int j = jj < 6 ? jj : 15;
        auto sg = [&](int kind, int r) { const int c = laser_slot_code<BOTH>(quad_laser_slot(kind, r, j)); return c >= 0 && (c & 64) != 0; };
        for (int r = 0; r < 6; ++r) {
            if (sg(1, r)) return false;
            if (sg(0, r) != (r < 2 ? sg(0, 0) : (r > 2 && sg(0, 3)))) return false;
            if (j < 6 && sg(2, r) != (r < 2 && sg(2, 0))) return false;
        }
        if (sg(0, 0) != sg(0, 1) || (j < 6 && sg(2, 0) != sg(2, 1))) return false;
    }
    return true;
}
static_assert(quad_sign_rows_ok<true>() && quad_sign_rows_ok<false>(), "sign rows of the laser reads");
template <bool BOTH> constexpr unsigned long long quad_code_pack(int kind, int r) {
    unsigned long long v = 0;
    for (int jj = 0; jj < 7; ++jj) {
        const int c = (kind == 2 && jj == 6) ? -1 : laser_slot_code<BOTH>(quad_laser_slot(kind, r, jj < 6 ? jj : 15));
        v |= (unsigned long long)(c < 0 ? 0xff : c) << (8 * jj);
    }
    return v;
}
template <int KIND, int R> __device__ __forceinline__ int quad_code(bool track, int role) {
    constexpr unsigned long long both = quad_code_pack<true>(KIND, R), one = quad_code_pack<false>(KIND, R);
    const int c = (int)(((track ? one : both) >> (8 * role)) & 0xffull);
    return c == 0xff ? -1 : c;
}
__device__ __forceinline__ double flip_sign(double x, unsigned m) { return __hiloint2double(__double2hiint(x) ^ (int)m, __double2loint(x)); }
constexpr int BSD2 = 3;
constexpr int QTOT_2 = BSD2 * (((4 * REC_GS + 127) / 128) * 128 + 6 * 32);
constexpr int QTOT = QTOT_1 > QTOT_2 ? QTOT_1 : QTOT_2;

template <int R> __device__ __forceinline__ int tri_rc(int j, int cj) {
    constexpr int cR = 14 * R - (R * (R - 1)) / 2;
    return R <= j ? cR + j : cj + R;
}

__global__ __launch_bounds__(64, 1) void k_lm_step_quad(StepArgs a) {
    __shared__ double S[QTOT];
    const int lane = threadIdx.x & 63, j = lane & 15, w = lane >> 4;
    const int n = a.n;
    const bool track = a.mode == LIW_MODE_TRACK;
    const int fast = a.fast_mode;
    auto is_const = [&](int i, int v) { return track && i < n - 1 && (v < 6 || (fast && v >= 9)); };
    int b = (int)blockIdx.x * 4 + w;
    bool act;
    const int* const alist = a.use_active ? usable_active_list(a.w.active, a.B) : nullptr;
    if (alist) {
        act = b < alist[0];
        b = act ? alist[1 + b] : 0;
        if ((unsigned)b >= (unsigned)a.B) { act = false; b = 0; }
    } else {
        act = b < a.B;
        b = act ? b : a.B - 1;
    }
    double* const X = a.x;
    double* const XC = a.w.x_cand;
    double* const LMD = reinterpret_cast<double*>(a.w.lm);
    constexpr unsigned LMS = sizeof(LmState) / 8, LM_SCALE = offsetof(LmState, scale) / 8, LM_DIAG = offsetof(LmState, diagonal) / 8,
                       LM_X0 = offsetof(LmState, x0) / 8;
    const unsigned oX = (unsigned)b * (unsigned)(n * 15), oLM = (unsigned)b * LMS;
    LmState& st = a.w.lm[b];
    act = act && !st.done;
    const int have_cand = st.have_candidate;
    {
        const double sl = quad_slow_lane(X + oX, XC + oX, have_cand, n, j, 16) ? 1.0 : 0.0;
        act = act && !(row_max(sl) > 0.0);
    }
    if (act && j == 0) st.pad_ = 1;
    if (!__any(act)) return;

    int reuse = st.reuse_diagonal, cur = st.cur;
    const int iteration = st.iteration;
    bool proceed = act, last_successful = true;
    const bool fresh = iteration == 0 && !have_cand;
    const bool clk_k = g_qclk_on[0] && (int)blockIdx.x == g_qclk_on[1] && iteration == g_qclk_on[3] && lane == 0;
    if (clk_k) g_qclk[12] = clock64();
    double inv_radius;
    {
        double radius = st.radius, dec = st.decrease_factor, x_cost = st.x_cost, x_norm = st.x_norm;
        const int max_iters = st.max_iters, successful0 = st.successful;
        int successful = successful0;
        const double model0 = st.model_cost_change, cand_step_norm = st.cand_step_norm, initial_cost0 = st.initial_cost;
        double minimum_cost = st.minimum_cost, initial_cost = initial_cost0;
        const int cb = (fresh || !have_cand) ? cur : 1 - cur;
        double cost;
        {
            const double* CSb = (cb ? a.w.CS[1] : a.w.CS[0]) + cs_index(n, b, 0, 0);
            double s = 0.0;
            for (int i = j; i < n; i += 16) {
                s += CSb[CS_LASER * n + i];
                if (!(track && i < n - 1)) s += CSb[CS_GROUND * n + i];
            }
            for (int k = j; k < n - 1; k += 16) {
                s += CSb[CS_IMU * n + k];
                if (!(track && k < n - 2)) s += CSb[CS_WHEEL * n + k];
            }
            if (track && !fast && a.has_prior[b] && j < 15) {
                const double* xs = ((fresh || !have_cand) ? X : XC) + oX + (unsigned)((n - 2) * 15);
                const double* pJ = a.prior_J + (size_t)b * 225 + j * 15;
                const double* pX = a.prior_X + (size_t)b * 15;
                double r = 0.0;
#pragma unroll
                for (int q = 0; q < 15; ++q) r += pJ[q] * (xs[q] - pX[q]);
                s += r * r;
            }
            cost = 0.5 * row_sum(s);
        }
        int term = 0;
        bool accept = false, fail_eval = false;
        if (fresh) {
            x_cost = cost; initial_cost = cost; minimum_cost = cost;
            fail_eval = !isfinite(cost);
        } else if (have_cand) {
            const double cand_cost = isfinite(cost) ? cost : kFailedEvalCost;
            term = lm_candidate_term(cand_step_norm, x_norm, x_cost, cand_cost);
            if (!term) {
                const double rho = (x_cost - cand_cost) / model0;
                accept = lm_accepts(rho);
                if (accept) {
                    cur = cb; x_cost = cand_cost;
                    lm_step_accepted(rho, radius, dec, reuse);
                    successful += 1;
                    if (x_cost < minimum_cost) minimum_cost = x_cost;
                } else {
                    lm_step_rejected(radius, dec, reuse);
                    last_successful = false;
                }
            }
        } else {
            last_successful = false;
        }
        {
            double s2 = 0.0;
            const bool restore = act && fail_eval && !fresh && successful0 > 0;
            const bool hist = act && a.w.history && iteration < a.w.history_records && !fail_eval;
            for (int e0 = j; e0 < n * 15; e0 += 16 * 8) {
                double xv[8];
#pragma unroll
                for (int q = 0; q < 8; ++q) {
                    const int e = e0 + 16 * q;
                    const unsigned ee = (unsigned)(e < n * 15 ? e : j);
                    xv[q] = restore ? LMD[oLM + LM_X0 + ee] : (accept ? XC[oX + ee] : X[oX + ee]);
                }
#pragma unroll
                for (int q = 0; q < 8; ++q) {
                    const int e = e0 + 16 * q;
                    if (e < n * 15) {
                        if (act && (accept || restore)) X[oX + (unsigned)e] = xv[q];
                        if (act && fresh) LMD[oLM + LM_X0 + (unsigned)e] = xv[q];
                        if (!is_const(e / 15, e % 15)) s2 += xv[q] * xv[q];
                        if (hist) a.w.history[((size_t)iteration * a.B + b) * (size_t)(n * 15) + e] = xv[q];
                    }
                }
            }
            s2 = row_sum(s2);
            if (fresh || accept) x_norm = sqrt(s2);
        }
        if (act && (fail_eval || term)) {
            if (j == 0) {
                st.done = 1; st.termination = fail_eval ? 6 : term;
                if (fail_eval) { st.x_cost = fresh ? cost : initial_cost0; st.have_candidate = 0; if (!fresh) st.iteration = iteration - 1; }
                if (fresh) { st.initial_cost = initial_cost; st.minimum_cost = minimum_cost; }
            }
            proceed = false;
        }
        const bool cap = proceed && lm_cap_reached(iteration, max_iters, fresh);
        if (proceed && j == 0) {
            st.radius = radius; st.decrease_factor = dec; st.x_cost = x_cost; st.x_norm = x_norm; st.cur = cur;
            st.successful = successful; st.minimum_cost = minimum_cost;
            if (fresh) st.initial_cost = initial_cost;
            if (cap) { st.done = 1; st.termination = 4; st.reuse_diagonal = reuse; st.have_candidate = 0; }
        }
        if (cap) proceed = false;
        inv_radius = 1.0 / radius;
    }
    if (!__any(proceed)) return;

    const double* const PL0 = a.w.PL[0];
    const double* const PI0 = a.w.PI[0];
    const double* const PW0 = a.w.PW[0];
    const double* const PG0 = a.w.PG[0];
    const unsigned oPL = (unsigned)b * (unsigned)(n * LPC) + (cur ? (unsigned)(a.w.PL[1] - a.w.PL[0]) : 0u);
    const unsigned oPI = (unsigned)b * (unsigned)(n * PIFS) + (cur ? (unsigned)(a.w.PI[1] - a.w.PI[0]) : 0u);
    const unsigned oPW = (unsigned)b * (unsigned)((n - 1) * PWS) + (cur ? (unsigned)(a.w.PW[1] - a.w.PW[0]) : 0u);
    const unsigned oPG = (unsigned)b * (unsigned)(n * PGS) + (cur ? (unsigned)(a.w.PG[1] - a.w.PG[0]) : 0u);
    const unsigned oWS = (unsigned)b * (unsigned)(n * SOLVE_WS);
    double* const WS = a.w.solve_ws;
    const unsigned oSC = oLM + LM_SCALE, oDG = oLM + LM_DIAG;
    const int jc = j < 15 ? j : 0;
    const bool l6 = j < 6, lm = j < 15;

    const bool prior_row = track && !fast && a.has_prior[b] != 0;
    if (__any(proceed && fresh)) {
        double sp = 0.0;
        if (prior_row) for (int k = 0; k < 15; ++k) { const double v = a.prior_J[(size_t)b * 225 + k * 15 + jc]; sp += v * v; }
        const int cbb = track ? laser_slot_code<false>(36 + (l6 ? jc : 0) * 7) : laser_slot_code<true>(36 + (l6 ? jc : 0) * 7);
        const int caa = track ? laser_slot_code<false>((l6 ? jc : 0) * 7) : laser_slot_code<true>((l6 ? jc : 0) * 7);
        for (int i0 = 0; i0 < n; i0 += 4) {
            double vbb[4], vjj[4], vii[4], vg[4], vi[4];
#pragma unroll
            for (int u = 0; u < 4; ++u) {
                const int i = min(i0 + u, n - 1);
                const int j6 = l6 ? jc : 0;
                vbb[u] = PL0[oPL + (unsigned)(i * LPC + (cbb >= 0 ? cbb & 63 : 0))];
                vbb[u] = cbb >= 0 ? vbb[u] : 0.0;
                vjj[u] = n > 1 ? PW0[oPW + (unsigned)(max(i - 1, 0) * PWS + PW_JJ(j6, j6))] : 0.0;
                vii[u] = n > 1 ? PW0[oPW + (unsigned)(min(i, n - 2) * PWS + PW_II(j6, j6))] : 0.0;
                vg[u] = PG0[oPG + (unsigned)(i * PGS + PG_H(j6, j6))];
                vi[u] = PI0[oPI + (unsigned)(i * PIFS + PIF_D + pi_tri(jc, jc))];
            }
#pragma unroll
            for (int u = 0; u < 4; ++u) {
                const int i = i0 + u;
                if (i >= n) break;
                double dd = 0.0;
                if (l6) {
                    dd += vbb[u];
                    if (i == 0) for (int f = 0; f < n; ++f) { const double va = PL0[oPL + (unsigned)(f * LPC + (caa >= 0 ? caa & 63 : 0))]; dd += caa >= 0 ? va : 0.0; }
                    if (i >= 1) dd += vjj[u];
                    if (i <= n - 2) dd += vii[u];
                    dd += vg[u];
                }
                if (n > 1) dd += vi[u];
                if (prior_row && i == n - 2) dd += sp;
                if (proceed && fresh && lm) LMD[oSC + (unsigned)(i * 15 + j)] = is_const(i, j) ? 1.0 : 1.0 / (1.0 + sqrt(dd));
            }
        }
    }
    const double sc0 = l6 ? LMD[oSC + (unsigned)jc] : 0.0;

    constexpr int S_IMU = 0, S_PL = 4 * PIFS, S_PW = S_PL + 4 * LPC, S_PG = S_PW + 4 * PWS, S_TR = S_PG + 4 * PGS + QPAD;
    constexpr int S_ZERO = S_TR + QTR, S_TAB = S_ZERO + QZB;
    static_assert(S_TAB + QTAB <= QTOT && 8 * QTOT < 65536, "LDS layout");
    const unsigned rPI[4] = {(unsigned)__builtin_amdgcn_readlane(oPI, 0), (unsigned)__builtin_amdgcn_readlane(oPI, 16), (unsigned)__builtin_amdgcn_readlane(oPI, 32), (unsigned)__builtin_amdgcn_readlane(oPI, 48)};
    const unsigned rPW[4] = {(unsigned)__builtin_amdgcn_readlane(oPW, 0), (unsigned)__builtin_amdgcn_readlane(oPW, 16), (unsigned)__builtin_amdgcn_readlane(oPW, 32), (unsigned)__builtin_amdgcn_readlane(oPW, 48)};
    const unsigned oPGw = oPG + (unsigned)(PG0 - PW0);
    const unsigned oPLw = oPL + (unsigned)(PL0 - PW0);
    const unsigned rPLw[4] = {(unsigned)__builtin_amdgcn_readlane(oPLw, 0), (unsigned)__builtin_amdgcn_readlane(oPLw, 16), (unsigned)__builtin_amdgcn_readlane(oPLw, 32), (unsigned)__builtin_amdgcn_readlane(oPLw, 48)};
    const unsigned rPGw[4] = {(unsigned)__builtin_amdgcn_readlane(oPGw, 0), (unsigned)__builtin_amdgcn_readlane(oPGw, 16), (unsigned)__builtin_amdgcn_readlane(oPGw, 32), (unsigned)__builtin_amdgcn_readlane(oPGw, 48)};
    typedef __attribute__((address_space(3))) void* lds_t;
    const int j_ = j;
    double scm_n = 1.0, dg_n = 0.0, xq_n = 0.0;
    auto prefetch_regs = [&](int f) {
        const int jq = j_ < 15 ? j_ : 0;
        scm_n = (j_ < 15 && f >= 1) ? LMD[oSC + (unsigned)((f - 1) * 15 + jq)] : 1.0;
        dg_n = LMD[oDG + (unsigned)(f * 15 + jq)];
        xq_n = X[oX + (unsigned)(f * 15 + jq)];
    };
    auto prefetch = [&](int f) {
        asm volatile("s_waitcnt lgkmcnt(0)" ::: "memory");
        const int k = f - 1;
        int lane2 = lane * 2;
        asm volatile("" : "+v"(lane2));
        if (n > 1) {
            sfor<0, 4>([&](auto W) {
                constexpr int ws = KI(W);
                const double* g = PI0 + rPI[ws] + (unsigned)(f * PIFS) + lane2;
                sfor<0, 3>([&](auto Q) { __builtin_amdgcn_global_load_lds(g, (lds_t)(S + S_IMU + ws * PIFS), 16, KI(Q) * 1024, 0); });
            });
        }
        {
            const unsigned fl = (unsigned)(f * LPC), fw = (unsigned)((k >= 0 ? k : 0) * PWS), fg = (unsigned)(f * PGS);
            constexpr int NPC = (4 * (LPC + PWS + PGS) + 127) / 128;
            static_assert(NPC * 128 - 4 * (LPC + PWS + PGS) <= QPAD && LPC % 2 == 0 && PWS % 2 == 0 && PGS % 2 == 0, "stream pieces: pad, 16-byte slots");
            sfor<0, NPC>([&](auto P) {
                constexpr int q0 = KI(P) * 128;
                unsigned off = 0;
                sfor<0, 12>([&](auto G) {
                    constexpr int g = KI(G);
                    constexpr int st = g < 4 ? g * LPC : g < 8 ? 4 * LPC + (g - 4) * PWS : 4 * (LPC + PWS) + (g - 8) * PGS;
                    constexpr int en = g == 11 ? (1 << 20) : st + (g < 4 ? LPC : g < 8 ? PWS : PGS);
                    if constexpr (st < q0 + 128 && en > q0) {
                        const unsigned v = (g < 4 ? rPLw[g & 3] + fl : g < 8 ? rPW[g & 3] + fw : rPGw[g & 3] + fg) + (unsigned)(lane2 - (st - q0));
                        if constexpr (st <= q0) off = v; else off = lane2 >= st - q0 ? v : off;
                    }
                });
                __builtin_amdgcn_global_load_lds(PW0 + off, (lds_t)(S + S_PL + q0), 16, 0, 0);
            });
        }
        asm volatile("" ::: "memory");
        prefetch_regs(f);
    };
    const double* SI = S + S_IMU + w * PIFS;
    unsigned short* const TAB = reinterpret_cast<unsigned short*>(S + S_TAB);
    {
        const int jt = j < 15 ? j : 0, cjt = 14 * jt - (jt * (jt - 1)) / 2, j6t = j < 6 ? j : 0;
        const bool t6 = j < 6, t15 = j == 15, tm = j < 15;
        const int oL = S_PL + w * LPC, oW_ = S_PW + w * PWS, oG = S_PG + w * PGS, oI = S_IMU + w * PIFS;
        auto put = [&](int k, bool on, int idx) { TAB[k * 64 + lane] = (unsigned short)(8 * (on ? idx : S_ZERO)); };
        const int role = t15 ? 6 : j6t;
        auto put_laser = [&](int k, bool on, int code) { put(k, on && code >= 0, oL + (code & 63)); };
        for (int e = lane; e < QZB; e += 64) S[S_ZERO + e] = 0.0;
        sfor<0, 6>([&](auto R) {
            constexpr int r = KI(R);
            put_laser(K_A + r, t6 || t15, quad_code<0, r>(track, role));
            put(K_B + r, t6 || t15, oW_ + (t15 ? PW_G(6 + r) : PW_JJ(r, j6t)));
            put(K_C + r, t6 || t15, oG + (t15 ? PG_G(r) : PG_H(r, j6t)));
            put_laser(K_HA + r, t6 || t15, quad_code<1, r>(track, role));
            put(K_CW + r, t6 || t15, oW_ + (t15 ? PW_G(r) : PW_II(r, j6t)));
            put_laser(K_RL + r, t6, quad_code<2, r>(track, role));
        });
        put(K_GSH, t6, oW_ + PW_G(j6t));
        sfor<0, 15>([&](auto R) {
            constexpr int r = KI(R);
            put(K_D + r, tm, oI + PIF_D + tri_rc<r>(jt, cjt));
        });
    }
    unsigned sgA0, sgA3, sgR0;
    {
        const bool t6 = j < 6, t15 = j == 15;
        const int role = t15 ? 6 : (t6 ? j : 0);
        const int cA0 = quad_code<0, 0>(track, role), cA3 = quad_code<0, 3>(track, role), cR0 = quad_code<2, 0>(track, role);
        sgA0 = ((t6 || t15) && cA0 >= 0 && (cA0 & 64)) ? 0x80000000u : 0u;
        sgA3 = ((t6 || t15) && cA3 >= 0 && (cA3 & 64)) ? 0x80000000u : 0u;
        sgR0 = (t6 && cR0 >= 0 && (cR0 & 64)) ? 0x80000000u : 0u;
    }
    const int lane_tab = lane * 2;
    auto RD = [&](auto K) -> double {
        constexpr int k = KI(K);
        const unsigned off = *reinterpret_cast<const unsigned short*>(reinterpret_cast<const char*>(TAB) + k * 128 + lane_tab);
        return *reinterpret_cast<const double*>(reinterpret_cast<const char*>(S) + off);
    };
    double* ST = S + S_TR + w * 90;

    double d[15], o[15], rr[15], cd[15], crt[6], D0[6], hA[6];
    double g0 = 0.0, gm = 0.0, ytg = 0.0, pdiag = 0.0, gsum = 0.0, gsh = 0.0;
    bool solved = true;
    sfor<0, 15>([&](auto R) { constexpr int r = KI(R); cd[r] = 0.0; });
    sfor<0, 6>([&](auto R) { D0[KI(R)] = 0.0; crt[KI(R)] = 0.0; hA[KI(R)] = 0.0; });
    const bool clk_on = g_qclk_on[0] && (int)blockIdx.x == g_qclk_on[1] && iteration == g_qclk_on[3];
    const int clk_frame = g_qclk_on[2];
    if (clk_k) g_qclk[13] = clock64();
    prefetch(n - 1);
    double sci_carry = (j_ < 15) ? LMD[oSC + (unsigned)((n - 1) * 15 + (j_ < 15 ? j_ : 0))] : 1.0;
    for (int i = n - 1; i >= 0; --i) {
        QSTAMP(0);
        int j = j_;
        asm volatile("" : "+v"(j));
        const int jc = j < 15 ? j : 0, j6 = j < 6 ? j : 0;
        const bool l6 = j < 6, l15 = j == 15, lm = j < 15;
        const bool hasm = i >= 1;
        asm volatile("s_waitcnt vmcnt(0)" ::: "memory");
        QSTAMP(1);
        const double sci = sci_carry, scm = scm_n, dg_old = dg_n, xq = xq_n;
        sci_carry = scm;
        const unsigned long long m15 = l15 ? ~0ull : 0ull, mh = hasm ? ~0ull : 0ull;
        double tS[6], oW[6], rL[6];
        {
            constexpr int NT = K_D - K_A;
            unsigned of[NT + 15], ofR[6];
            auto tab_at = [&](int k) { return (unsigned)*reinterpret_cast<const unsigned short*>(reinterpret_cast<const char*>(TAB) + k * 128 + lane_tab); };
            sfor<0, NT>([&](auto Q) { constexpr int q = KI(Q); of[q] = tab_at(K_A + q); });
            sfor<0, 6>([&](auto Q) { constexpr int q = KI(Q); ofR[q] = tab_at(K_RL + q); });
            if (n > 1) sfor<0, 15>([&](auto Q) { constexpr int q = KI(Q); of[NT + q] = tab_at(K_D + q); });
            const char* const Sb = reinterpret_cast<const char*>(S);
            const int w8 = (lane >> 4) * 8;
            const char* const bOV = Sb + (l15 ? 8 * (S_IMU + PIF_GJ) : 8 * (S_IMU + PIF_IJ) + jc * 120) + w8 * PIFS;
            const char* const bGI = Sb + (l15 ? 8 * (S_IMU + PIF_GI) + w8 * PIFS : 8 * S_ZERO);
            const char* const bOW = Sb + (l6 ? 8 * (S_PW + PW_IJ(0, 0)) + w8 * PWS + j6 * 48 : 8 * S_ZERO);
            double gi[15];
            if (n > 1) {
                sfor<0, 15>([&](auto R) { constexpr int r = KI(R); o[r] = *reinterpret_cast<const double*>(bOV + 8 * r); gi[r] = *reinterpret_cast<const double*>(bGI + 8 * r); });
            } else {
                sfor<0, 15>([&](auto R) { constexpr int r = KI(R); d[r] = 0.0; o[r] = 0.0; gi[r] = 0.0; });
            }
            sfor<0, 6>([&](auto R) { constexpr int r = KI(R); oW[r] = *reinterpret_cast<const double*>(bOW + 8 * r); });
            asm volatile("" ::: "memory");
            double pb[NT];
            sfor<0, NT>([&](auto Q) { constexpr int q = KI(Q); pb[q] = *reinterpret_cast<const double*>(Sb + of[q]); });
            sfor<0, 6>([&](auto R) { constexpr int r = KI(R); rL[r] = *reinterpret_cast<const double*>(Sb + ofR[r]); });
            if (n > 1) sfor<0, 15>([&](auto Q) { constexpr int q = KI(Q); d[q] = *reinterpret_cast<const double*>(Sb + of[NT + q]); });
            asm volatile("" ::: "memory");
            pb[K_A + 0] = flip_sign(pb[K_A + 0], sgA0); pb[K_A + 1] = flip_sign(pb[K_A + 1], sgA0);
            pb[K_A + 3] = flip_sign(pb[K_A + 3], sgA3); pb[K_A + 4] = flip_sign(pb[K_A + 4], sgA3); pb[K_A + 5] = flip_sign(pb[K_A + 5], sgA3);
            rL[0] = flip_sign(rL[0], sgR0); rL[1] = flip_sign(rL[1], sgR0);
            sfor<0, 6>([&](auto R) { constexpr int r = KI(R); tS[r] = pb[K_A + r] + bits_and(pb[K_B + r], mh) + pb[K_C + r]; });
            if (!track) {
                sfor<0, 6>([&](auto R) { constexpr int r = KI(R); hA[r] += pb[K_HA + r]; });
                if (i == 0) sfor<0, 6>([&](auto R) { tS[KI(R)] += hA[KI(R)]; });
            }
            sfor<0, 15>([&](auto R) { constexpr int r = KI(R); o[r] = bits_and(o[r], mh) + gi[r]; });
        }
        sfor<0, 15>([&](auto R) { rr[KI(R)] = 0.0; });
        sfor<0, 6>([&](auto R) {
            constexpr int r = KI(R);
            d[r] += bits_and(tS[r], ~m15);
            o[r] += bits_and(tS[r], m15) + bits_and(oW[r], mh);
            rr[r] = bits_and(rL[r], mh);
        });
        if (track && i == n - 2 && __any(prior_row)) {
            double Jc[15];
            const double dxl = (lm && prior_row) ? X[oX + (unsigned)((n - 2) * 15 + jc)] - a.prior_X[(size_t)b * 15 + jc] : 0.0;
            sfor<0, 15>([&](auto K) { constexpr int k = KI(K); Jc[k] = (lm && prior_row) ? a.prior_J[(size_t)b * 225 + k * 15 + jc] : 0.0; });
            double gp = 0.0;
            sfor<0, 15>([&](auto K) { constexpr int k = KI(K); const double rp = row_sum(Jc[k] * dxl); gp = __builtin_fma(Jc[k], rp, gp); });
            dpp_fence();
            sfor<0, 15>([&](auto R) {
                constexpr int r = KI(R);
                sfor<0, 15>([&](auto K) { constexpr int k = KI(K); fnma_bc<r>(d[r], Jc[k], -Jc[k]); });
                const double gr = bc<r>(gp);
                o[r] += l15 ? gr : 0.0;
            });
        }
        QSTAMP(2);
        QSTAMP(3);
        {
            double* GT = const_cast<double*>(SI) + PIF_IJ;
            if (l15) sfor<0, 15>([&](auto R) { constexpr int r = KI(R); GT[r] = o[r]; });
            const double gt = gsh + (lm ? GT[jc] : 0.0);
            double m = fabs(gt);
            {
                const double av = xq - gt;
                const double a2 = mul_nop(av, av);
                const double s2 = bc<3>(a2) + bc<4>(a2) + bc<5>(a2);
                if (__any(proceed && !(s2 < 9.8))) {
                    dpp_fence();
                    const V3<double> nq = normalize_so3(V3<double>(bc<3>(av), bc<4>(av), bc<5>(av)));
                    if (j == 3) m = fabs(xq - nq.x);
                    if (j == 4) m = fabs(xq - nq.y);
                    if (j == 5) m = fabs(xq - nq.z);
                }
            }
            if (!lm || is_const(i, j)) m = 0.0;
            gm = fmax(gm, m);
            gsum += lm ? gt : 0.0;
        }
        double dmp;
        {
            double mjj = d[0];
            sfor<1, 15>([&](auto R) { constexpr int r = KI(R); mjj = (j == r) ? d[r] : mjj; });
            double dgv = dg_old;
            if (!reuse) {
                dgv = fmin(fmax(__builtin_fma(mjj, sci * sci, pdiag), kMinDiag), kMaxDiag);
                if (proceed && lm) LMD[oDG + (unsigned)(i * 15 + j)] = dgv;
            }
            dmp = dgv * inv_radius;
        }
        QSTAMP(4);
        dpp_fence();
        const double* const stp = (l6 && i < n - 1) ? ST + j6 : S + S_ZERO;
        sfor<0, 15>([&](auto R) {
            constexpr int r = KI(R);
            const double rs = bc<r>(sci);
            d[r] = __builtin_fma(d[r], rs * sci, cd[r]) + ((j == r) ? dmp : 0.0);
            o[r] = __builtin_fma(o[r], rs * scm, bits_and(cd[r], m15));
            rr[r] = __builtin_fma(rr[r], rs * sc0, stp[r * 6]);
        });
        if (i == 1) {
            sfor<0, 15>([&](auto R) { constexpr int r = KI(R); o[r] += rr[r]; rr[r] = 0.0; });
        }
        if (i == 0) {
            dpp_fence();
            sfor<0, 6>([&](auto R) {
                constexpr int r = KI(R);
                const double gr = bc<r>(g0);
                d[r] += D0[r];
                o[r] += l15 ? gr : 0.0;
            });
        }
        if (track) {
            const bool colc = lm && is_const(i, j);
            const bool nbc = lm && hasm && is_const(i - 1, j);
            sfor<0, 15>([&](auto R) {
                constexpr int r = KI(R);
                const bool rowc = is_const(i, r);
                if (rowc || colc) d[r] = (j == r) ? 1.0 : 0.0;
                if (rowc || nbc) o[r] = 0.0;
                if (rowc) rr[r] = 0.0;
            });
        }
        QSTAMP(5);
        if (hasm) {
            dpp_fence();
            double cw[6];
            sfor<0, 6>([&](auto R) { constexpr int r = KI(R); cw[r] = RD(KC<K_CW + r>{}); });
            gsh = RD(KC<K_GSH>{});
            __builtin_amdgcn_sched_barrier(0);
            sfor<0, 15>([&](auto R) {
                constexpr int r = KI(R);
                double fi = 0.0;
                if constexpr (r < 6) {
                    const double rs = bc<r>(scm);
                    fi = cw[r] * (rs * scm);
                }
                cd[r] = fi;
                pdiag = (j == r) ? cd[r] : pdiag;
            });
        } else {
            gsh = 0.0;
        }
        sfor<0, 6>([&](auto Q) { crt[KI(Q)] = 0.0; });
        if (i >= 1) prefetch(i - 1);
        QSTAMP(6);
        sfor<0, 15>([&](auto K) {
            constexpr int k = KI(K);
            const double piv = bc<k>(d[k]);
            if (k == 14) solved = solved && (piv > 0.0) && isfinite(piv);
            const double inv = fast_rsqrt(piv);
            const double wkd = mul_nop(d[k], inv);
            const double wko = o[k] * inv, wkr = rr[k] * inv;
            d[k] = l15 ? inv : wkd;
            o[k] = wko; rr[k] = wkr;
            sfor<k + 1, 15>([&](auto R) {
                constexpr int r = KI(R);
                fnma_bc<r>(d[r], wkd, wkd);
                fnma_bc<r>(o[r], wkd, wko);
                fnma_bc<r>(rr[r], wkd, wkr);
            });
        });
        QSTAMP(7);
        sfor<0, 15>([&](auto K) { constexpr int k = KI(K); ytg = __builtin_fma(o[k], o[k], ytg); });
        if (hasm) {
            dpp_fence();
            sfor<0, 15>([&](auto K) {
                constexpr int k = KI(K);
                sfor<0, 15>([&](auto C) { constexpr int c = KI(C); fnma_bc<c>(cd[c], o[k], o[k]); });
            });
            if (i >= 2) {
                sfor<0, 15>([&](auto K) {
                    constexpr int k = KI(K);
                    sfor<0, 6>([&](auto Q) { constexpr int q = KI(Q); fnma_bc<q>(crt[q], rr[k], o[k]); });
                    sfor<0, 6>([&](auto C) { constexpr int c = KI(C); fnma_bc<c>(D0[c], rr[k], rr[k]); });
                    fnma_bc<15>(g0, o[k], rr[k]);
                });
            }
            if (lm) sfor<0, 6>([&](auto Q) { constexpr int q = KI(Q); ST[jc * 6 + q] = crt[q]; });
        }
        QSTAMP(8);
        dpp_fence();
        sfor<0, 15>([&](auto T_) {
            constexpr int r = 14 - KI(T_);
            const double ir = bc<15>(d[r]);
            o[r] *= ir; rr[r] *= ir;
            sfor<0, r>([&](auto K) {
                constexpr int k = KI(K);
                fnma_bc<r>(o[k], d[k], o[r]);
                fnma_bc<r>(rr[k], d[k], rr[r]);
            });
        });
        QSTAMP(9);
        if (proceed) {
            const unsigned of = oWS + (unsigned)(i * SOLVE_WS);
            sfor<0, 15>([&](auto K) {
                constexpr int k = KI(K);
                WS[of + (unsigned)(k * REC_LD + (l15 ? 21 : j))] = o[k];
                if (l6) WS[of + (unsigned)(k * REC_LD + 15 + j)] = rr[k];
            });
        }
        QSTAMP(10);
    }
    if (clk_k) g_qclk[14] = clock64();
    dpp_fence();
    const double gmax = row_max(gm);
    ytg = bc<15>(ytg);
    {
// ... 77 lines not shown
        const double* const rowp = B_ + w * REC_GS + jc * REC_LD;
        double row[22];
        sfor<0, 11>([&](auto K) { constexpr int k = KI(K); const double2 v = reinterpret_cast<const double2*>(rowp)[k]; row[2 * k] = v.x; row[2 * k + 1] = v.y; });
        const double xold = B_[RECP * 128 + w * 15 + jc], scv = B_[RECP * 128 + XP * 32 + w * 15 + jc], dgv = B_[RECP * 128 + XP * 32 + 60 + w * 15 + jc];
        double t = row[21];
        dpp_fence();
        if (i >= 1) sfor<0, 15>([&](auto K) { constexpr int k = KI(K); fnma_bc<k>(t, yprev, row[k]); });
        if (i >= 2) sfor<0, 6>([&](auto K) { constexpr int k = KI(K); fnma_bc<k>(t, y0v, row[15 + k]); });
        yprev = t;
        if (i == 0) y0v = t;
        const bool cst = is_const(i, j);
        const double del = (lm && !cst) ? -t * scv : 0.0;
        double xnew = xold + del;
        {
            dpp_fence();
            const double a0 = bc<3>(xnew), a1 = bc<4>(xnew), a2 = bc<5>(xnew);
            if (!is_const(i, 3) && __any(proceed && !(a0 * a0 + a1 * a1 + a2 * a2 < 9.8))) {
                const V3<double> nq = normalize_so3(V3<double>(a0, a1, a2));
                if (j == 3) xnew = nq.x;
                if (j == 4) xnew = nq.y;
                if (j == 5) xnew = nq.z;
            }
        }
        if (lm) {
            if (proceed) XC[oX + (unsigned)(i * 15 + j)] = xnew;
            if (!cst) {
                sn2 += (xold - xnew) * (xold - xnew);
                dsum += dgv * inv_radius * t * t;
            }
        }
    };
    sfor<0, BSD2>([&](auto Q) { constexpr int q = KI(Q); if (q < n) stage2(q, q); });
    for (int i0 = 0; i0 < n; i0 += BSD2) {
        sfor<0, BSD2>([&](auto Q) {
            constexpr int q = KI(Q);
            __builtin_amdgcn_sched_barrier(0);
            const int i = i0 + q;
            if (i < n) {
                const int later = min(n - 1 - i, BSD2 - 1);
                if (later >= 2) asm volatile("s_waitcnt vmcnt(%0)" ::"n"(2 * NLD) : "memory");
                else if (later == 1) asm volatile("s_waitcnt vmcnt(%0)" ::"n"(NLD) : "memory");
                else asm volatile("s_waitcnt vmcnt(0)" ::: "memory");
                solve_frame(q, i);
                if (i + BSD2 < n) stage2(i + BSD2, q);
            }
        });
    }
    if (clk_k) g_qclk[15] = clock64();
    const double step_norm = sqrt(row_sum(sn2));
    const double model_cost_change = 0.5 * (ytg + row_sum(dsum));
    const bool valid = lm_step_valid(solved, model_cost_change);
    const int invalid0 = st.invalid_steps, successful = st.successful;
    const bool fail5 = !valid && lm_gives_up(invalid0);
    if (proceed && fail5 && successful > 0) {
        for (int e = j; e < n * 15; e += 16) X[oX + (unsigned)e] = LMD[oLM + LM_X0 + (unsigned)e];
    }
    if (proceed && j == 0) {
        double radius = st.radius, dec = st.decrease_factor;
        st.iteration = iteration + 1;
        if (fail5 && successful > 0) st.x_cost = st.initial_cost;
        if (valid) {
            st.reuse_diagonal = 1;
            st.model_cost_change = model_cost_change; st.cand_step_norm = step_norm; st.have_candidate = 1; st.invalid_steps = 0;
        } else {
            st.invalid_steps = invalid0 + 1;
            st.have_candidate = 0;
            if (fail5) { st.done = 1; st.termination = 6; st.iteration = iteration; }
            lm_step_rejected(radius, dec, reuse);
            st.radius = radius; st.decrease_factor = dec; st.reuse_diagonal = reuse;
        }
    }
}

bool lm_step_quad_fits(const StepArgs& a) {
    const unsigned long long lim = 0xFFFFFFFFull - 4096;
    auto span = [&](const double* p0, const double* p1, unsigned long long per) {
        const unsigned long long d = p1 >= p0 ? (unsigned long long)(p1 - p0) : ~0ull;
        return d <= lim && d + (unsigned long long)a.B * per <= lim;
    };
    const int nm = a.n > 1 ? a.n - 1 : 1;
    return a.n >= 1 && (a.mode == LIW_MODE_INIT || (a.mode == LIW_MODE_TRACK && a.n >= 2)) && span(a.w.PL[0], a.w.PL[1], (unsigned long long)a.n * LPC) && a.w.pi_frame && a.w.pl_compact &&
           a.w.PL[0] >= a.w.PW[0] && span(a.w.PW[0], a.w.PL[1], (unsigned long long)a.n * LPC) &&
           a.w.CS[0] && a.w.CS[1] && span(a.w.PI[0], a.w.PI[1], (unsigned long long)a.n * PIFS) &&
           span(a.w.PW[0], a.w.PW[1], (unsigned long long)nm * PWS) && span(a.w.PG[0], a.w.PG[1], (unsigned long long)a.n * PGS) &&
           a.w.PG[0] >= a.w.PW[0] && span(a.w.PW[0], a.w.PG[1], (unsigned long long)a.n * PGS) &&
           (unsigned long long)a.B * (sizeof(LmState) / 8) <= lim && (unsigned long long)a.B * a.n * SOLVE_WS <= lim;
}
extern "C" void liw_debug_quad_clk(int on, int block, int frame, int iteration, long long* out) {
    const int v[4] = {on, block, frame, iteration};
    (void)hipMemcpyToSymbol(HIP_SYMBOL(g_qclk_on), v, sizeof(v));
    if (out) (void)hipMemcpyFromSymbol(out, HIP_SYMBOL(g_qclk), sizeof(long long) * 64);
}
void launch_lm_step_quad(const StepArgs& a, hipStream_t s) {
    hipLaunchKernelGGL(k_lm_step_quad, dim3((a.B + 3) / 4), dim3(64), 0, s, a);
}

}
```

### 2dliw-slam_amd/csrc/liw_capi.hip

```cpp
#include <hip/hip_runtime.h>

#include <algorithm>
#include <cmath>
#include <cstdio>
#include <cstdlib>
#include <atomic>
#include <chrono>
#include <cstring>
#include <string>
#include <vector>

#include "liw_host_common.hpp"
#include "liw_kernels.hpp"

using namespace liw;

struct DevBuf {
    void* p = nullptr;
    size_t cap = 0;
    int ensure(size_t bytes) {
        if (bytes <= cap && p) return 0;
        if (p) (void)hipFree(p);
        p = nullptr; cap = 0;
        if (hipMalloc(&p, bytes ? bytes : 8) != hipSuccess) return -1;
// ... 115 lines not shown
    dp->ground_p_info = 1.0 / prm->manifold_p_sigma;
    dp->ground_q_info = 1.0 / prm->manifold_q_sigma;
    dp->fast_mode = prm->fast_mode;
}

extern "C" {

liw_ctx* liw_create(const liw_params* prm) {
    if (!prm) return nullptr;
    liw_ctx* c = new liw_ctx();
    c->prm = *prm;
    liw_fill_devparams(prm, &c->dp);
    int ndev = 0;
    if (hipGetDeviceCount(&ndev) == hipSuccess && ndev > prm->device && prm->device >= 0) {
        hipDeviceProp_t props;
        if (hipSetDevice(prm->device) == hipSuccess && hipGetDeviceProperties(&props, prm->device) == hipSuccess) {
            if (std::strstr(props.gcnArchName, "gfx950") != nullptr) {
                if (hipStreamCreate(&c->stream) == hipSuccess) c->have_device = true;
                if (c->have_device && hipStreamCreateWithFlags(&c->fork.side[0], hipStreamNonBlocking) == hipSuccess &&
                    hipStreamCreateWithFlags(&c->fork.side[1], hipStreamNonBlocking) == hipSuccess &&
                    hipEventCreateWithFlags(&c->fork.ev_fork, hipEventDisableTiming) == hipSuccess &&
                    hipEventCreateWithFlags(&c->fork.ev_join[0], hipEventDisableTiming) == hipSuccess &&
                    hipEventCreateWithFlags(&c->fork.ev_join[1], hipEventDisableTiming) == hipSuccess &&
                    hipEventCreateWithFlags(&c->fork.ev_compact, hipEventDisableTiming) == hipSuccess)
                    c->have_fork = true;
                if (std::getenv("LIW_SERIAL_ROLES")) c->have_fork = false;
                if (std::getenv("LIW_NO_SPEC_MARG")) c->spec_marg = false;
                if (std::getenv("LIW_NO_REATTACH")) c->reattach = false;
                (void)hipEventCreateWithFlags(&c->ev_upload, hipEventDisableTiming);
            } else {
                c->err = std::string("device is ") + props.gcnArchName + ", this library is built for gfx950 only";
            }
        }
    }
    if (!c->have_device && c->err.empty()) c->err = "no HIP device";
    return c;
}

void liw_destroy(liw_ctx* c) {
    if (!c) return;
    if (c->have_device) {
        (void)hipSetDevice(c->prm.device);
        DevBuf* bufs[] = {&c->lpk, &c->lpk_off, &c->lpk_mx, &c->lpk_perm, &c->p2p_err, &c->arena, &c->prior_X, &c->prior_J, &c->prior_R, &c->has_prior, &c->ws, &c->scratch,
                          &c->priorn_X, &c->priorn_J, &c->priorn_R, &c->has_priorn, &c->result, &c->marg_status};
        if (c->pinned) (void)hipHostFree(c->pinned);
        if (c->rb_pin) (void)hipHostFree(c->rb_pin);
        if (c->ev_upload) (void)hipEventDestroy(c->ev_upload);
        for (DevBuf* b : bufs) b->release();
        for (auto e : c->ev_lin) (void)hipEventDestroy(e);
        for (auto e : c->ev_step) (void)hipEventDestroy(e);
        for (auto e : c->ev_x) (void)hipEventDestroy(e);
        if (c->gexec) (void)hipGraphExecDestroy(c->gexec);
        if (c->have_fork) {
            (void)hipStreamDestroy(c->fork.side[0]); (void)hipStreamDestroy(c->fork.side[1]);
            (void)hipEventDestroy(c->fork.ev_fork); (void)hipEventDestroy(c->fork.ev_join[0]); (void)hipEventDestroy(c->fork.ev_join[1]); (void)hipEventDestroy(c->fork.ev_compact);
        }
        if (c->stream) (void)hipStreamDestroy(c->stream);
    }
    delete c;
}

const char* liw_last_error(const liw_ctx* c) { return c ? c->err.c_str() : "null ctx"; }

int liw_get_extrinsics(const liw_ctx* c, double* A, double* Bm) {
    if (!c) return LIW_EINVAL;
    auto put = [](const double* R, const double* t, double* m) {
        for (int i = 0; i < 3; ++i) { for (int j = 0; j < 3; ++j) m[i * 4 + j] = R[i * 3 + j]; m[i * 4 + 3] = t[i]; }
        m[12] = m[13] = m[14] = 0.0; m[15] = 1.0;
    };
    if (A) put(c->dp.Riw, c->dp.tiw, A);
    if (Bm) put(c->dp.Ril, c->dp.til, Bm);
    return LIW_OK;
}

struct FullLayout {
    size_t PL[2], PI[2], PW[2], PG[2], CS[2], x_cand, group_off, lm, solve_ws, info, history, active, imu_pk, imu_pk_bad, bytes;
};
static FullLayout full_layout(int B, int n, int hist) {
    FullLayout f{};
    size_t o = 0;
    const int nm = n > 1 ? n - 1 : 1;
    const int lps = laser_stride(pi_frame_format(B) ? 1 : 0);
    for (int k = 0; k < 2; ++k) { f.PI[k] = o; o = al256(o + sizeof(double) * (size_t)B * pi_doubles_per_window(n)); }
    for (int k = 0; k < 2; ++k) { f.PW[k] = o; o = al256(o + sizeof(double) * (size_t)B * nm * PWS); }
    for (int k = 0; k < 2; ++k) { f.PL[k] = o; o = al256(o + sizeof(double) * (size_t)B * n * lps); }
    for (int k = 0; k < 2; ++k) { f.PG[k] = o; o = al256(o + sizeof(double) * (size_t)B * n * PGS); }
    f.x_cand = o; o = al256(o + sizeof(double) * (size_t)B * n * 15);
    f.group_off = o; o = al256(o + sizeof(int) * (size_t)B * (n + 1));
    f.active = o; o = al256(o + compact_list_bytes_host(B));
    f.lm = o; o = al256(o + sizeof(LmState) * (size_t)B);
    f.solve_ws = o; o = al256(o + sizeof(double) * (size_t)B * n * SOLVE_WS);
    f.info = o; o = al256(o + sizeof(liw_summary) * (size_t)B);
    f.history = hist > 0 ? o : 0;
    if (hist > 0) o = al256(o + sizeof(double) * (size_t)hist * B * n * 15);
    f.imu_pk_bad = o; o = al256(o + 2 * sizeof(int));
    f.imu_pk = o; o = al256(o + sizeof(double) * (size_t)B * nm * IMU_PK);
    for (int k = 0; k < 2; ++k) { f.CS[k] = o; o = al256(o + sizeof(double) * (size_t)B * 4 * n); }
    f.bytes = o;
    return f;
}
static WsView make_view(void* ws, int B, int n, int hist) {
    FullLayout f = full_layout(B, n, hist);
    char* base = (char*)ws;
    WsView v{};
    for (int k = 0; k < 2; ++k) {
        v.PL[k] = (double*)(base + f.PL[k]); v.PI[k] = (double*)(base + f.PI[k]);
        v.PW[k] = (double*)(base + f.PW[k]); v.PG[k] = (double*)(base + f.PG[k]);
    }
    v.x_cand = (double*)(base + f.x_cand);
    v.group_off = (int*)(base + f.group_off);
    v.lm = (LmState*)(base + f.lm);
    v.solve_ws = (double*)(base + f.solve_ws);
    v.info = (liw_summary*)(base + f.info);
    v.history = hist > 0 ? (double*)(base + f.history) : nullptr;
    v.history_records = hist;
    v.active = (int*)(base + f.active);
    v.pi_frame = pi_frame_format(B) ? 1 : 0;
    v.pl_compact = v.pi_frame;
    for (int k = 0; k < 2; ++k) v.CS[k] = (double*)(base + f.CS[k]);
    v.imu_pk = (double*)(base + f.imu_pk);
    v.imu_pk_bad = (int*)(base + f.imu_pk_bad);
    return v;
}

int liw_batch_ws_layout(int B, int n, int history_records, liw_ws_layout* out) {
    if (!out || B <= 0 || n <= 0 || n > 64) return LIW_EINVAL;
    FullLayout f = full_layout(B, n, history_records);
    out->bytes = f.bytes;
    out->laser_partial_off[0] = f.PL[0];
    out->laser_partial_off[1] = f.PL[1];
    out->laser_partial_stride = laser_stride(pi_frame_format(B) ? 1 : 0);
    out->laser_partial_bytes = sizeof(double) * (size_t)B * n * out->laser_partial_stride;
    out->info_off = f.info;
    out->history_off = f.history;
    return LIW_OK;
}

static int check_batch(liw_ctx* c, const liw_batch* b, int min_n = 1) {
    if (!b || b->B <= 0 || b->n <= 0 || b->n > 64) return fail(c, LIW_EINVAL, "bad batch (need 1 <= n <= 64, B >= 1)");
    if (b->n < min_n) return fail(c, LIW_EINVAL, "TRACK / MARG topology needs n >= 2 (the prior block is tied to frame n-2)");
    return LIW_OK;
}
static int min_frames(int mode) { return mode == LIW_MODE_INIT ? 1 : 2; }
static bool lpk_matches(const liw_ctx* c, const liw_batch* b, const void* ws) {
    return c && c->lpk_on && c->lpk_key.ws == ws && c->lpk_key.pts == b->laser_pts && c->lpk_key.frame == b->laser_frame && c->lpk_key.B == b->B &&
           c->lpk_key.n == b->n && c->lpk_key.Ltot == (long)b->Ltot;
}
static int laser_slab_begin(liw_ctx* c, const liw_batch* b, int mode, const WsView& v, void* ws, hipStream_t s, bool may_sync) {
    c->lpk_on = false;
    if (!may_sync || std::getenv("LIW_NO_LASER_SLAB")) return LIW_OK;
    const int S = laser_slab_count(b->B), N = S * b->n;
    if ((mode == LIW_MODE_INIT ? N < 2048 : S < 256) || b->Ltot <= 0) return LIW_OK;
    if (c->lpk_mx.ensure(sizeof(int) * (size_t)N) || c->lpk_off.ensure(sizeof(long long) * ((size_t)N + 2)) || c->lpk_perm.ensure(sizeof(int) * (size_t)N * 64))
        return fail(c, LIW_ENOMEM, "hipMalloc");
    launch_laser_slab_prepare(b->B, b->n, v.group_off, c->lpk_perm.as<int>(), c->lpk_mx.as<int>(), c->lpk_off.as<long long>(), v.imu_pk_bad + 1, s);
    if (!c->rb_pin) HIPCHK(c, hipHostMalloc((void**)&c->rb_pin, 64, hipHostMallocDefault));
    long long* const tail = reinterpret_cast<long long*>(c->rb_pin) + 2;
    tail[0] = 0; tail[1] = 1;
    HIPCHK(c, hipMemcpyAsync(tail, c->lpk_off.as<long long>() + N, 2 * sizeof(long long), hipMemcpyDeviceToHost, s));
    HIPCHK(c, hipStreamSynchronize(s));
    const long long rows = tail[0];
    if (tail[1] != 0 || rows <= 0) return LIW_OK;
    if (rows * 64 > 4 * (long long)b->Ltot + 64ll * N) return LIW_OK;
    if (c->lpk.ensure(sizeof(double) * LASER_SLAB_ROWD * (size_t)rows)) { c->lpk.release(); return LIW_OK; }
    launch_laser_slab_pack(b->B, b->n, (long)b->Ltot, v.group_off, c->lpk_perm.as<int>(), b->laser_pts, c->lpk_off.as<long long>(), c->lpk_mx.as<int>(), c->lpk.as<double>(), s);
    c->lpk_key = {ws, b->laser_pts, b->laser_frame, b->B, b->n, (long)b->Ltot};
    c->lpk_on = true;
    c->lpk_rows = rows;
    return LIW_OK;
}
static LinArgs lin_args(const liw_batch* b, int mode, const double* x, const WsView& v, int candidate, bool use_lm, bool packed = false, const liw_ctx* c = nullptr, const void* ws = nullptr) {
    LinArgs A{};
    A.B = b->B; A.n = b->n; A.mode = mode; A.eval_small = b->eval_small;
    A.x = x; A.group_off = v.group_off; A.laser_off = b->laser_off; A.laser_pts = b->laser_pts; A.Ltot = b->Ltot;
    A.match_pose = b->match_pose; A.has_match = b->has_match;
    A.imu_X = b->imu_X; A.imu_J = b->imu_J; A.imu_sqrtP = b->imu_sqrtP; A.imu_Dt = b->imu_Dt;
    A.wheel_T = b->wheel_T; A.wheel_sqrtP = b->wheel_sqrtP;
    for (int k = 0; k < 2; ++k) { A.PL[k] = v.PL[k]; A.PI[k] = v.PI[k]; A.PW[k] = v.PW[k]; A.PG[k] = v.PG[k]; }
    A.lm = use_lm ? v.lm : nullptr;
    A.active = use_lm ? v.active : nullptr;
    A.candidate = candidate;
    A.pi_frame = v.pi_frame;
    A.pl_compact = v.pl_compact;
    for (int k = 0; k < 2; ++k) A.CS[k] = v.pi_frame ? v.CS[k] : nullptr;
    if (packed && b->n > 1 && b->eval_small) { A.imu_pk = v.imu_pk; A.imu_pk_bad = v.imu_pk_bad; }
    if (packed) A.laser_hz = v.imu_pk_bad + 1;
    if (packed && lpk_matches(c, b, ws)) { A.laser_pk = c->lpk.as<double>(); A.laser_slab_off = c->lpk_off.as<long long>(); A.laser_perm = c->lpk_perm.as<int>(); }
    return A;
}
static StepArgs step_args(liw_ctx* c, const liw_batch* b, int mode, int max_iters, const WsView& v) {
    StepArgs a{};
    a.B = b->B; a.n = b->n; a.mode = mode; a.max_iters = max_iters; a.fast_mode = c->prm.fast_mode;
    a.x = b->x; a.match_pose = b->match_pose; a.has_match = b->has_match;
    a.prior_X = b->prior_X; a.prior_J = b->prior_J; a.has_prior = b->has_prior;
    a.w = v;
    a.use_active = lin_builds_active_list(b->B, b->eval_small) ? 1 : 0;
    return a;
}
static int resolve_iters(liw_ctx* c, int mode, int max_iters) {
    if (max_iters > 0) return max_iters;
    return (mode == LIW_MODE_TRACK && c->prm.fast_mode) ? 10 : 50;
}


int liw_batch_lm_begin(liw_ctx* c, const liw_batch* b, int mode, int max_iters, void* ws, void* stream) {
    NEEDDEV(c);
    if (int r = check_batch(c, b, min_frames(mode))) return r;
    c->last_iters = resolve_iters(c, mode, max_iters);
    WsView v = make_view(ws, b->B, b->n, b->history_records);
    hipStream_t s = (hipStream_t)stream;
    launch_group_offsets(b->B, b->n, b->laser_off, b->laser_frame, v.group_off, s);
    launch_lm_begin(b->B, b->n, v.lm, c->last_iters, s);
    (void)hipMemsetAsync(v.active + b->B + 1, 0, compact_list_bytes_host(b->B) - sizeof(int) * ((size_t)b->B + 1), s);
    if (b->n > 1 && b->eval_small) {
        if ((long)b->B * (b->n - 1) >= 4096 && !std::getenv("LIW_NO_IMU_PACK"))
            launch_imu_pack(b->B, b->n, b->imu_X, b->imu_J, b->imu_sqrtP, b->imu_Dt, v.imu_pk, v.imu_pk_bad, s);
        else (void)hipMemsetAsync(v.imu_pk_bad, 0xff, sizeof(int), s);
    }
    if ((long)b->B * (b->n - 1) >= 4096) {
        launch_laser_z_scan(b->Ltot, b->laser_pts, v.imu_pk_bad + 1, s);
        hipStreamCaptureStatus cap = hipStreamCaptureStatusNone;
        (void)hipStreamIsCapturing(s, &cap);
        if (int r = laser_slab_begin(c, b, mode, v, ws, s, cap == hipStreamCaptureStatusNone)) return r;
    } else {
        (void)hipMemsetAsync(v.imu_pk_bad + 1, 0xff, sizeof(int), s);
        c->lpk_on = false;
    }
    HIPCHK(c, hipGetLastError());
    return LIW_OK;
}
int liw_batch_launch_paths(liw_ctx* c, const liw_batch* b, const void* ws, int* flags) {
    if (!c) return LIW_EINVAL;
    if (int r = check_batch(c, b)) return r;
    if (!flags) return fail(c, LIW_EINVAL, "liw_batch_launch_paths: null flags");
    *flags = (pi_frame_format(b->B) ? 1 : 0) | (lpk_matches(c, b, ws) ? 2 : 0);
    return LIW_OK;
}
int liw_batch_packed_rows(liw_ctx* c, const liw_batch* b, const void* ws, long long* rows, long long* blocks) {
    if (!c) return LIW_EINVAL;
    if (int r = check_batch(c, b)) return r;
    if (rows) *rows = lpk_matches(c, b, ws) ? c->lpk_rows : 0;
    if (blocks) *blocks = (long long)b->Ltot;
    return LIW_OK;
}
int liw_batch_lm_linearize(liw_ctx* c, const liw_batch* b, int mode, int candidate, void* ws, void* stream) {
    NEEDDEV(c);
    if (int r = check_batch(c, b, min_frames(mode))) return r;
    WsView v = make_view(ws, b->B, b->n, b->history_records);
    LinArgs A = lin_args(b, mode, candidate ? v.x_cand : b->x, v, candidate != 0, true, true, c, ws);
    launch_linearize(A, c->dp, (hipStream_t)stream, c->have_fork ? &c->fork : nullptr);
    HIPCHK(c, hipGetLastError());
    return LIW_OK;
}
int liw_batch_lm_linearize_async(liw_ctx* c, const liw_batch* b, int mode, int candidate, void* ws, void* stream) {
    NEEDDEV(c);
    if (int r = check_batch(c, b, min_frames(mode))) return r;
    WsView v = make_view(ws, b->B, b->n, b->history_records);
    LinArgs A = lin_args(b, mode, candidate ? v.x_cand : b->x, v, candidate != 0, true, true, c, ws);
    launch_linearize(A, c->dp, (hipStream_t)stream, c->have_fork ? &c->fork : nullptr, true);
    HIPCHK(c, hipGetLastError());
    return LIW_OK;
}
int liw_batch_lm_join(liw_ctx* c, void* stream) {
    NEEDDEV(c);
    launch_linearize_join((hipStream_t)stream, c->have_fork ? &c->fork : nullptr);
    HIPCHK(c, hipGetLastError());
// ... 778 lines not shown
```

### 2dliw-slam_amd/csrc/liw_kernels.hpp

```cpp
#pragma once
#include <cstdlib>
#include <hip/hip_runtime.h>
#include <stdint.h>

#include "../../include/liw_window.h"
#include "liw_dual.hpp"
#include "liw_lm_rules.hpp"

namespace liw {

struct DevParams {
    double Riw[9], tiw[3];
    double Ril[9], til[3];
    double g;
    double laser_sqrt_info;
    double ground_p_info;
    double ground_q_info;
    int fast_mode;
};

constexpr int LP = LIW_LASER_PARTIAL;
constexpr int PIS = 496;
constexpr int PI_II = 0, PI_IJ = 120, PI_JJ = 345, PI_G = 465, PI_C = 495;
__host__ __device__ inline int pi_tri(int r, int c) {
    const int lo = r < c ? r : c, hi = r < c ? c : r;
    return lo * 15 - (lo * (lo - 1)) / 2 + (hi - lo);
}
constexpr int PIF_D = 0, PIF_IJ = 120, PIF_GJ = 345, PIF_GI = 360, PIF_C = 375, PIFS = 376;
constexpr int QUAD_MIN_BATCH = 1024;
enum StepVariant { STEP_AUTO = -1, STEP_LATENCY = 0, STEP_THROUGHPUT = 1, STEP_TWO_WAVE = 2, STEP_QUAD = 3, STEP_DENSE2 = 4 };
inline StepVariant forced_step_variant() {
    const char* env = getenv("LIW_STEP_VARIANT");
    if (!env) return STEP_AUTO;
    return env[0] >= '1' && env[0] <= '4' ? (StepVariant)(env[0] - '0') : STEP_LATENCY;
}
inline bool step_variant_is(StepVariant forced, StepVariant v, bool by_size) { return forced == STEP_AUTO ? by_size : forced == v; }
inline bool pi_frame_format(int B, StepVariant forced = forced_step_variant()) { return step_variant_is(forced, STEP_QUAD, B >= QUAD_MIN_BATCH); }
__host__ __device__ inline size_t pi_doubles_per_window(int n) {
    const size_t a = (size_t)(n > 1 ? n - 1 : 1) * PIS, b = (size_t)n * PIFS;
    return a > b ? a : b;
}
template <int N> __host__ __device__ constexpr int tri_sym(int r, int c) {
    return r <= c ? r * N - (r * (r - 1)) / 2 + (c - r) : c * N - (c * (c - 1)) / 2 + (r - c);
}
constexpr int CS_LASER = 0, CS_GROUND = 1, CS_IMU = 2, CS_WHEEL = 3;
__host__ __device__ inline size_t cs_index(int n, int b, int role, int rec) { return ((size_t)b * 4 + role) * n + rec; }
constexpr int PWS = 92;
__host__ __device__ constexpr int PW_II(int r, int c) { return tri_sym<6>(r, c); }
__host__ __device__ constexpr int PW_IJ(int r, int c) { return 21 + r * 6 + c; }
__host__ __device__ constexpr int PW_JJ(int r, int c) { return 57 + tri_sym<6>(r, c); }
__host__ __device__ constexpr int PW_G(int e) { return 78 + e; }
constexpr int PW_C = 90;
constexpr int PGS = 28;
__host__ __device__ constexpr int PG_H(int r, int c) { return tri_sym<7>(r, c); }
__host__ __device__ constexpr int PG_G(int r) { return tri_sym<7>(r, 6); }
constexpr int PG_C = 27;
constexpr int FTF = 32;

struct LmState {
    double radius, decrease_factor, x_cost, x_norm, minimum_cost;
    double cand_step_norm, model_cost_change;
    int reuse_diagonal, iteration, done, termination, successful, cur, invalid_steps, have_candidate;
    int max_iters, pad_;
    double initial_cost;
    double scale[15 * 64];
    double diagonal[15 * 64];
    double x0[15 * 64];
};

__device__ __forceinline__ void lm_reset(LmState& s, int max_iters) {
    s.radius = kInitRadius; s.decrease_factor = 2.0; s.x_cost = 0.0; s.x_norm = 0.0; s.minimum_cost = 0.0;
    s.cand_step_norm = 0.0; s.model_cost_change = 0.0; s.reuse_diagonal = 0; s.iteration = 0; s.done = 0; s.termination = 0;
    s.successful = 0; s.cur = 0; s.invalid_steps = 0; s.have_candidate = 0; s.initial_cost = 0.0; s.max_iters = max_iters; s.pad_ = 0;
}

struct WsView {
    double* PL[2]; double* PI[2]; double* PW[2]; double* PG[2];
    double* x_cand;
    int* group_off;
    LmState* lm;
    double* solve_ws;
    liw_summary* info;
    double* history;
    int history_records;
    int* active;
    int pi_frame;
    int pl_compact;
    double* CS[2];
    double* imu_pk;
    int* imu_pk_bad;
};
constexpr int IMU_PK = 192, IPK_DT = 15, IPK_J = 16, IPK_S = 70;
constexpr int REC_LD = 22;
constexpr int REC_GS = 15 * REC_LD;
constexpr int SOLVE_WS = REC_GS + 16;

struct LinArgs {
    int B, n, mode, eval_small;
    const double* x;
    const int* group_off;
    const int* laser_off;
    const double* laser_pts; int Ltot;
    const double* match_pose;
    const unsigned char* has_match;
    const double* imu_X; const double* imu_J; const double* imu_sqrtP; const double* imu_Dt;
    const double* wheel_T; const double* wheel_sqrtP;
    double* PL[2]; double* PI[2]; double* PW[2]; double* PG[2];
    const LmState* lm;
    const LmState* gate;
    LmState* reset_lm;
    int reset_iters;
    int marg_older;
    int candidate;
    int small_per_wave;
    int imu_per_wave;
    int small_nd;
    int* active;
    int pi_frame;
    int pl_compact;
    double* CS[2];
    const double* imu_pk;
    const int* imu_pk_bad;
    const int* laser_hz;
    const double* laser_pk;
    const long long* laser_slab_off;
    const int* laser_perm;
    int role_mask;
    double* dbg_laser_res; double* dbg_laser_jac; double* dbg_imu_res; double* dbg_imu_jac;
    double* dbg_wheel_res; double* dbg_wheel_jac; double* dbg_ground_res; double* dbg_ground_jac;
};

template <bool BOTH> constexpr int laser_pairidx(int c1, int c2) {
    constexpr int NC = BOTH ? 9 : 6;
    return c1 > c2 ? laser_pairidx<BOTH>(c2, c1) : c1 * NC - c1 * (c1 - 1) / 2 + (c2 - c1);
}
constexpr int laser_col_a(int idx) { return idx < 2 ? idx : (idx == 2 ? -1 : idx - 1); }
template <bool BOTH> constexpr int laser_col_b(int idx) { return BOTH ? (idx < 2 ? idx : (idx == 2 ? -1 : idx + 2)) : (idx == 2 ? -1 : (idx < 2 ? idx : idx - 1)); }
template <bool BOTH> constexpr bool laser_neg_b(int idx) { return BOTH && idx < 2; }
template <bool BOTH>
__host__ __device__ constexpr int laser_slot_code(int s) {
    constexpr int RC = (BOTH ? 9 : 6) - 1;
    int src = -1;
    bool neg = false;
    if (s < 0) {
    } else if (s < 36) {
        const int ca = laser_col_a(s / 6), cb = laser_col_a(s % 6);
        if (BOTH && ca >= 0 && cb >= 0) src = laser_pairidx<BOTH>(ca, cb);
    } else if (s < 72) {
        const int ia = (s - 36) / 6, ib = (s - 36) % 6, ca = laser_col_b<BOTH>(ia), cb = laser_col_b<BOTH>(ib);
        if (ca >= 0 && cb >= 0) { src = laser_pairidx<BOTH>(ca, cb); neg = laser_neg_b<BOTH>(ia) != laser_neg_b<BOTH>(ib); }
    } else if (s < 108) {
        const int ia = (s - 72) / 6, ib = (s - 72) % 6, ca = laser_col_a(ia), cb = laser_col_b<BOTH>(ib);
        if (BOTH && ca >= 0 && cb >= 0) { src = laser_pairidx<BOTH>(ca, cb); neg = laser_neg_b<BOTH>(ib); }
    } else if (s < 114) {
        const int ca = laser_col_a(s - 108);
        if (BOTH && ca >= 0) src = laser_pairidx<BOTH>(ca, RC);
    } else if (s < 120) {
        const int cb = laser_col_b<BOTH>(s - 114);
        if (cb >= 0) { src = laser_pairidx<BOTH>(cb, RC); neg = laser_neg_b<BOTH>(s - 114); }
    } else if (s == 120) {
        src = laser_pairidx<BOTH>(RC, RC);
    }
    return src < 0 ? -1 : (src | (neg ? 64 : 0));
}
template <bool BOTH> __host__ __device__ constexpr bool laser_slot_zero(int s) { return laser_slot_code<BOTH>(s) < 0; }
constexpr int LPC = LIW_LASER_PARTIAL_COMPACT;
__host__ __device__ constexpr int laser_stride(int compact) { return compact ? LPC : LP; }
constexpr int LPC_COST_BOTH = laser_pairidx<true>(8, 8), LPC_COST_ONE = laser_pairidx<false>(5, 5);
static_assert(laser_slot_code<true>(120) == LPC_COST_BOTH && laser_slot_code<false>(120) == LPC_COST_ONE && LPC_COST_BOTH == 44 && LPC_COST_ONE == 20, "cost total");
template <bool BOTH> __host__ __device__ inline double laser_slot(const double* rec, int s, int compact) {
    if (!compact) return rec[s];
    const int code = laser_slot_code<BOTH>(s);
    if (code < 0) return 0.0;
    const double v = rec[code & 63];
    return (code & 64) ? -v : v;
}
__host__ __device__ inline double laser_slot(const double* rec, int s, int compact, bool both) {
    return both ? laser_slot<true>(rec, s, compact) : laser_slot<false>(rec, s, compact);
}
struct LaserPackTable { short slot[45]; unsigned char neg[45]; };

__device__ __forceinline__ void lds_sync() {
    __builtin_amdgcn_fence(__ATOMIC_RELEASE, "wavefront");
    __builtin_amdgcn_wave_barrier();
    __builtin_amdgcn_fence(__ATOMIC_ACQUIRE, "wavefront");
}
__device__ __forceinline__ void wave_mem_sync() {
    __builtin_amdgcn_fence(__ATOMIC_RELEASE, "workgroup");
    __builtin_amdgcn_wave_barrier();
    __builtin_amdgcn_fence(__ATOMIC_ACQUIRE, "workgroup");
}

template <typename T> __device__ __forceinline__ void nt_store(T* p, T v) { __builtin_nontemporal_store(v, p); }

__device__ __forceinline__ double fast_rsqrt(double x) {
    double y = __builtin_amdgcn_rsq(x);
    const double hx = 0.5 * x;
    y = y * __builtin_fma(-hx, y * y, 1.5);
    y = y * __builtin_fma(-hx, y * y, 1.5);
    return y;
}
__device__ __forceinline__ double fast_rcp(double x) {
// ... 100 lines not shown
```

Measured before the change: 142,000 solves/s.

## Fold wheel and ground factor contributions into per-frame pose records

Adds a pose-fold format. The wheel/ground linearization kernel pre-sums the wheel II/JJ/IJ blocks and the ground Hessian and gradient into one 64-double record per frame, with costs written to the CS buffers. The assembly, diagonal, cost and quad-step LM kernels then read one record per frame instead of combining three separate wheel and ground records with hasm/hasp branching. This cuts global reads and per-frame additions in the hot LM step. In exchange the linearization kernel does more work, with a new wave-to-window mapping and cross-block reads in LDS. The format is on by default and can be disabled with an environment variable.

Result: no change. 143,700 solves/s (median of 2 runs) (+1.2%).

```diff
diff --git a/2dliw-slam_amd/csrc/k_linearize.hip b/2dliw-slam_amd/csrc/k_linearize.hip
--- a/2dliw-slam_amd/csrc/k_linearize.hip
+++ b/2dliw-slam_amd/csrc/k_linearize.hip
@@ -742,7 +742,34 @@
 constexpr int WG_PER_WAVE = 31, WG_REC = 68;
 constexpr int WG_LDS = WG_PER_WAVE * WG_REC + 96;
 __device__ __forceinline__ LJN<4> ext4(const J3& a) { LJN<4> r; r.v = a.v; r.d[0] = a.d[0]; r.d[1] = a.d[1]; r.d[2] = a.d[2]; r.d[3] = 0.0; return r; }
-template <bool COSTCOPY>
+__host__ __device__ inline int fold_parts(int nb) { return nb <= WG_PER_WAVE ? 1 : (nb + WG_PER_WAVE - 2) / (WG_PER_WAVE - 1); }
+__host__ __device__ inline int fold_windows(int nb, int pw) {
+    const int lim = pw < WG_PER_WAVE ? pw : WG_PER_WAVE;
+    return (nb >= 1 && lim >= nb) ? lim / nb : 1;
+}
+__host__ __device__ inline int fold_wave_count(int B, int n, int pw) {
+    const int nb = n - 1, parts = fold_parts(nb);
+    if (parts > 1) return B * parts;
+    const int wpw = fold_windows(nb, pw);
+    return (B + wpw - 1) / wpw;
+}
+struct PoseRcTab { int e[PPS]; };
+constexpr PoseRcTab make_pose_rc() {
+    PoseRcTab t{};
+    for (int e = 0; e < PPS; ++e) {
+        if (e < PP_G) {
+            int r = 0, q = e;
+            while (q >= 6 - r) { q -= 6 - r; ++r; }
+            t.e[e] = (r << 8) | (r + q);
+        } else if (e < PP_G + 6) t.e[e] = ((e - PP_G) << 8) | 6;
+        else if (e < PP_IJ) t.e[e] = 2 << 16;
+        else t.e[e] = (1 << 16) | (((e - PP_IJ) / 6) << 8) | ((e - PP_IJ) % 6);
+    }
+    return t;
+}
+__constant__ PoseRcTab c_pose_rc = make_pose_rc();
+static_assert(PP_H(5, 5) == PP_G - 1 && PP_G + 6 < PP_IJ && PP_IJ + 36 == PPS && PPS == 64, "pose record: two entries per lane of a half wave");
+template <bool COSTCOPY, bool FOLD = false>
 __device__ __forceinline__ void wheel_ground2_blocks(const LinArgs& A, const DevParams& P, int wave, double* lds, const int* const act) {
     typedef LJN<4> J4;
     typedef LJN<6> J6;
@@ -750,7 +777,26 @@
     const int n = A.n, nb = n - 1;
     const long total = (long)(act ? act[0] : A.B) * nb, gb = (long)wave * A.small_per_wave + blk;
     bool on = blk < A.small_per_wave && blk < WG_PER_WAVE && gb < total;
-    const int wi = on ? (int)(gb / nb) : 0, k = on ? (int)(gb % nb) : 0;
+    int wi = on ? (int)(gb / nb) : 0, k = on ? (int)(gb % nb) : 0;
+    int fold_slots = 0, fold_own = 0;
+    if constexpr (FOLD) {
+        const int cnt = act ? act[0] : A.B, parts = fold_parts(nb);
+        if (parts == 1) {
+            const int wpw = fold_windows(nb, A.small_per_wave), w0 = wave * wpw;
+            if (w0 >= cnt) return;
+            fold_own = fold_slots = min(wpw, cnt - w0) * nb;
+            on = blk < fold_slots;
+            wi = on ? w0 + blk / nb : 0; k = on ? blk % nb : 0;
+        } else {
+            const int bpw = (nb + parts - 1) / parts, part = wave % parts, kfirst = part * bpw, kend = min(nb, kfirst + bpw);
+            if (wave / parts >= cnt || kfirst >= kend) return;
+            fold_own = kend - kfirst;
+            fold_slots = fold_own + (kend < nb ? 1 : 0);
+            on = blk < fold_slots;
+            wi = on ? wave / parts : 0; k = on ? kfirst + blk : 0;
+        }
+    }
+    const bool slot_on = on;
     const int b = act ? act[1 + wi] : wi;
     if (on && !act) on = window_live(A, b);
     double* Y = lds + (blk < WG_PER_WAVE ? blk : 0) * WG_REC;
@@ -884,6 +930,57 @@
         meta[160 + blk] = k;
     }
     lds_sync();
+    if constexpr (FOLD) {
+        const double mult = (double)n;
+        const int mq = lane < WG_PER_WAVE ? lane : 0;
+        const int selv = meta[mq], csv = meta[64 + mq], cgv = meta[128 + mq], kv = meta[160 + mq];
+        const int half = lane >> 5, l2 = lane & 31;
+        const int eX = l2 < 27 ? l2 : (l2 < 31 ? 56 + 2 * (l2 - 27) : PP_G + 6), eA = l2 < 27 ? PP_IJ + l2 : 55 + 2 * (l2 - 27);
+        const int cX_ = c_pose_rc.e[eX], cA_ = c_pose_rc.e[eA];
+        const int kindX = cX_ >> 16, rX = (cX_ >> 8) & 255, cX = cX_ & 255, rA = (cA_ >> 8) & 255, cA = cA_ & 255;
+        const int a1 = kindX == 0 ? 6 + rX : rX, b1 = kindX == 0 ? (cX < 6 ? 6 + cX : 12) : 6 + cX;
+        const int a2 = kindX == 0 ? rX : 0, b2 = kindX == 0 ? (cX < 6 ? cX : 12) : 0;
+        const int a3 = kindX == 0 ? rX : 0, b3 = kindX == 0 ? cX : 0;
+        const int aA = rA, bA = 6 + cA;
+        auto dot3 = [](const double* Yq, int a, int c) { return __builtin_fma(Yq[26 + a], Yq[26 + c], __builtin_fma(Yq[a], Yq[c], Yq[13 + a] * Yq[13 + c])); };
+        for (int pass = 0; pass < 2; ++pass) {
+            if (pass == 1 && __builtin_amdgcn_ballot_w64(lane < fold_own && kv == 0) == 0) break;
+            for (int q = half; q < fold_own; q += 2) {
+                const int sel = meta[q], kq = meta[160 + q];
+                const size_t fq = (size_t)meta[96 + q] + (pass ? 0 : 1);
+                const double* Yq = lds + q * WG_REC;
+                const bool nxt = kq + 1 < nb;
+                const double* Yg = Yq + (pass ? 53 : 39);
+                const double u1 = dot3(Yq, a1, b1);
+                const double u2 = dot3((pass == 0 && nxt) ? Yq + WG_REC : Yq, a2, b2);
+                const double u3 = mult * __builtin_fma(Yg[7 + a3], Yg[7 + b3], Yg[a3] * Yg[b3]);
+                const double uA = dot3(Yq, aA, bA);
+                double vX, vA;
+                if (pass == 0) {
+                    const double d = (nxt ? u1 + u2 : u1) + u3;
+                    vX = kindX == 0 ? d : (kindX == 1 ? u1 : 0.0);
+                    vA = uA;
+                } else {
+                    vX = kindX == 0 ? u2 + u3 : 0.0;
+                    vA = 0.0;
+                }
+                if (sel >= 0 && (pass == 0 || kq == 0)) {
+                    double* rec = (sel ? A.PP[1] : A.PP[0]) + fq * PPS;
+                    rec[eX] = vX;
+                    rec[eA] = vA;
+                }
+            }
+        }
+        if (COSTCOPY && A.CS[0] && lane < fold_own && selv >= 0) {
+            const double* Yq = lds + lane * WG_REC;
+            double* CSb = selv ? A.CS[1] : A.CS[0];
+            CSb[csv] = __builtin_fma(Yq[38], Yq[38], __builtin_fma(Yq[12], Yq[12], Yq[25] * Yq[25]));
+            CSb[cgv + 1] = mult * __builtin_fma(Yq[39 + 13], Yq[39 + 13], Yq[39 + 6] * Yq[39 + 6]);
+            if (kv == 0) CSb[cgv] = mult * __builtin_fma(Yq[53 + 13], Yq[53 + 13], Yq[53 + 6] * Yq[53 + 6]);
+        }
+        (void)slot_on; (void)fold_slots;
+        return;
+    }
     const long gb0 = (long)wave * A.small_per_wave;
     const int nblk = (int)min((long)min(A.small_per_wave, WG_PER_WAVE), total - gb0);
     const int ml = lane < WG_PER_WAVE ? lane : 0;
@@ -1019,7 +1116,8 @@
     __shared__ double lds[WG_LDS > SMALL_LDS ? WG_LDS : SMALL_LDS];
     static_assert(sizeof(double) * (WG_LDS > SMALL_LDS ? WG_LDS : SMALL_LDS) * 4 * SMALL_OCC <= 160 * 1024, "LDS of the waves of a CU");
     const int* const act = usable_active_list(A.active, A.B);
-    if (A.n > 1) wheel_ground2_blocks<true>(A, P, (int)blockIdx.x, lds, act);
+    if (A.n > 1 && A.pose_fold) wheel_ground2_blocks<true, true>(A, P, (int)blockIdx.x, lds, act);
+    else if (A.n > 1) wheel_ground2_blocks<true>(A, P, (int)blockIdx.x, lds, act);
     else ground_frames<true>(A, P, (int)blockIdx.x, lds, act);
 }
 __global__ void k_lm_reset(int B, LmState* lm, int max_iters) {
@@ -1165,7 +1263,7 @@
     auto role_small = [&]() {
         if (!(small_waves && (rm & 4))) return;
         if (A.small_per_wave == WHEEL_PER_WAVE) A.small_per_wave = WG_PER_WAVE;
-        const int waves = n > 1 ? wheel_wave_count(B, n, A.small_per_wave) : ground_wave_count(B, n);
+        const int waves = n > 1 ? (A.pose_fold ? fold_wave_count(B, n, A.small_per_wave) : wheel_wave_count(B, n, A.small_per_wave)) : ground_wave_count(B, n);
         hipLaunchKernelGGL(k_lin_small, dim3((unsigned)waves), dim3(64), 0, s_small, A, P);
     };
     static const char* order_env = getenv("LIW_LIN_ORDER");
diff --git a/2dliw-slam_amd/csrc/k_lm.hip b/2dliw-slam_amd/csrc/k_lm.hip
--- a/2dliw-slam_amd/csrc/k_lm.hip
+++ b/2dliw-slam_amd/csrc/k_lm.hip
@@ -32,17 +32,20 @@
     int pif;
     int plc;
     const double* PL; const double* PI; const double* PW; const double* PG;
+    int ppf;
+    const double* PP; const double* CS;
     const double* x;
     const double* pJ; const double* pX; bool prior_on;
 };
 __device__ __forceinline__ AsmCtx asm_ctx(const WsView& w, int n, int mode, int fast, int b, const double* prior_J, const double* prior_X, bool prior_on) {
     AsmCtx c;
-    c.pif = w.pi_frame; c.plc = w.pl_compact; c.n = n; c.mode = mode; c.fast = fast; c.b = b;
+    c.pif = w.pi_frame; c.plc = w.pl_compact; c.ppf = w.pose_fold; c.n = n; c.mode = mode; c.fast = fast; c.b = b;
     c.pJ = prior_J + (size_t)b * 225; c.pX = prior_X + (size_t)b * 15; c.prior_on = prior_on;
     return c;
 }
 __device__ __forceinline__ void bind(AsmCtx& c, const WsView& w, int buf, const double* x) {
     c.buf = buf; c.PL = w.PL[buf]; c.PI = w.PI[buf]; c.PW = w.PW[buf]; c.PG = w.PG[buf]; c.x = x;
+    c.PP = w.PP[buf]; c.CS = w.CS[buf];
 }
 
 __device__ __forceinline__ void copy_states(double* dst, const double* src, int n, int lane) {
@@ -121,6 +124,10 @@
     const double* PLi = PLb + (size_t)i * LPS;
     const double* PL1 = PLb + (size_t)(n > 1 ? 1 : 0) * LPS;
     const double* PGi = PGb + (size_t)i * PGS;
+    const bool ppf = c.ppf != 0;
+    const double* PPb = c.PP + (size_t)c.b * n * PPS;
+    const double* PPi = PPb + (size_t)i * PPS;
+    const double* PPp = PPb + (size_t)(hasp ? i + 1 : i) * PPS;
     AsmRegs R;
 #pragma unroll
     for (int q = 0; q < 4; ++q) {
@@ -136,20 +143,22 @@
         const bool pl = lane < 36;
         const int r = pl ? lane / 6 : 0, cc = pl ? lane % 6 : 0;
         R.t1 = pl_slot(c, PLi, 36 + r * 6 + cc);
-        R.t2 = PWm[(unsigned)PW_JJ(r, cc)];
-        R.t3 = PWp[(unsigned)PW_II(r, cc)];
-        R.t4 = PGi[(unsigned)PG_H(r, cc)];
-        R.t8 = up ? PWp[(unsigned)PW_IJ(cc, r)] : PWm[(unsigned)PW_IJ(r, cc)];
-        R.e2 = up ? PWm[(unsigned)PW_IJ(r, cc)] : 0.0;
+        const double* const Wm = ppf ? PPi : PWm;
+        const double* const Wp = ppf ? PPp : PWp;
+        R.t2 = Wm[(unsigned)(ppf ? PP_H(r, cc) : PW_JJ(r, cc))];
+        R.t3 = ppf ? 0.0 : PWp[(unsigned)PW_II(r, cc)];
+        R.t4 = ppf ? 0.0 : PGi[(unsigned)PG_H(r, cc)];
+        R.t8 = up ? Wp[(unsigned)(ppf ? PP_IJ + cc * 6 + r : PW_IJ(cc, r))] : Wm[(unsigned)(ppf ? PP_IJ + r * 6 + cc : PW_IJ(r, cc))];
+        R.e2 = up ? Wm[(unsigned)(ppf ? PP_IJ + r * 6 + cc : PW_IJ(r, cc))] : 0.0;
         R.t9 = pl_slot(c, PL1, 72 + r * 6 + cc);
         R.t10 = pl_slot(c, PLi, 72 + r * 6 + cc);
     }
     {
         const int r = lane < 15 ? lane : 0, r6 = r < 6 ? r : 0;
         R.g1 = pl_slot(c, PLi, 114 + r6);
-        R.g2 = PWm[(unsigned)PW_G(6 + r6)];
-        R.g3 = PWp[(unsigned)PW_G(r6)];
-        R.g4 = PGi[(unsigned)PG_G(r6)];
+        R.g2 = (ppf ? PPi : PWm)[(unsigned)(ppf ? PP_G + r6 : PW_G(6 + r6))];
+        R.g3 = ppf ? 0.0 : PWp[(unsigned)PW_G(r6)];
+        R.g4 = ppf ? 0.0 : PGi[(unsigned)PG_G(r6)];
         R.g5 = PIm[(unsigned)((pif ? PIF_GJ : PI_G + 15) + r)];
         R.g6 = pif ? PIm[(unsigned)(PIF_GI + r)] : PIp[(unsigned)(PI_G + r)];
     }
@@ -220,7 +229,8 @@
     {
         const bool pl = lane < 36;
         const int r = pl ? lane / 6 : 0, cc = pl ? lane % 6 : 0;
-        dP = R.t1 + (hasm ? R.t2 : 0.0) + (hasp ? R.t3 : 0.0) + R.t4;
+        if (c.ppf) dP = R.t1 + R.t2;
+        else dP = R.t1 + (hasm ? R.t2 : 0.0) + (hasp ? R.t3 : 0.0) + R.t4;
         if (i == 0 && c.mode == LIW_MODE_INIT) {
             double s0 = 0.0, s1 = 0.0, s2 = 0.0, s3 = 0.0;
             int j = 0;
@@ -239,7 +249,8 @@
     {
         const int r = lane < 15 ? lane : 0;
         if (r < 6) {
-            gg = R.g1 + (hasm ? R.g2 : 0.0) + (hasp ? R.g3 : 0.0) + R.g4;
+            if (c.ppf) gg = R.g1 + R.g2;
+            else gg = R.g1 + (hasm ? R.g2 : 0.0) + (hasp ? R.g3 : 0.0) + R.g4;
             if (i == 0 && c.mode == LIW_MODE_INIT) {
                 double s0 = 0.0, s1 = 0.0, s2 = 0.0, s3 = 0.0;
                 int j = 0;
@@ -361,13 +372,18 @@
     for (int i = lane; i < n; i += 64) {
         const bool gon = !(track && i < n - 1);
         if (gon) s += pl_slot(c, PLb + (size_t)i * LPS, 120);
-        if (gon) s += PGb[(size_t)i * PGS + PG_C];
+        if (gon) s += c.ppf ? c.CS[cs_index(n, c.b, CS_GROUND, i)] : PGb[(size_t)i * PGS + PG_C];
         if (gchk) {
             if (gon) {
 #pragma unroll
                 for (int k = 0; k < 12; ++k) gs += pl_slot(c, PLb + (size_t)i * LPS, 108 + k);
             }
-            if (gon) {
+            if (c.ppf) {
+                if (!track || i >= n - 2) {
+#pragma unroll
+                    for (int k = 0; k < 6; ++k) gs += c.PP[((size_t)c.b * n + i) * PPS + PP_G + k];
+                }
+            } else if (gon) {
 #pragma unroll
                 for (int k = 0; k < 6; ++k) gs += PGb[(size_t)i * PGS + PG_G(k)];
             }
@@ -376,12 +392,12 @@
     for (int k = lane; k < n - 1; k += 64) {
         s += pif ? PIb[(size_t)(k + 1) * PIFS + PIF_C] : PIb[(size_t)k * PIS + PI_C];
         const bool won = !(track && k < n - 2);
-        if (won) s += PWb[(size_t)k * PWS + PW_C];
+        if (won) s += c.ppf ? c.CS[cs_index(n, c.b, CS_WHEEL, k)] : PWb[(size_t)k * PWS + PW_C];
         if (gchk) {
 #pragma unroll
             for (int e = 0; e < 30; ++e)
                 gs += pif ? (e < 15 ? PIb[(size_t)k * PIFS + PIF_GI + e] : PIb[(size_t)(k + 1) * PIFS + PIF_GJ + e - 15]) : PIb[(size_t)k * PIS + PI_G + e];
-            if (won) {
+            if (won && !c.ppf) {
 #pragma unroll
                 for (int e = 0; e < 12; ++e) gs += PWb[(size_t)k * PWS + PW_G(e)];
             }
@@ -487,9 +503,12 @@
     if (r < 6) {
         d += pl_slot(c, PLb + (size_t)i * LPS, 36 + r * 7);
         if (i == 0) for (int j = 0; j < n; ++j) d += pl_slot(c, PLb + (size_t)j * LPS, r * 7);
-        if (i >= 1) d += PWb[(size_t)(i - 1) * PWS + PW_JJ(r, r)];
-        if (i <= n - 2) d += PWb[(size_t)i * PWS + PW_II(r, r)];
-        d += PGb[(size_t)i * PGS + PG_H(r, r)];
+        if (c.ppf) d += c.PP[((size_t)c.b * n + i) * PPS + PP_H(r, r)];
+        else {
+            if (i >= 1) d += PWb[(size_t)(i - 1) * PWS + PW_JJ(r, r)];
+            if (i <= n - 2) d += PWb[(size_t)i * PWS + PW_II(r, r)];
+            d += PGb[(size_t)i * PGS + PG_H(r, r)];
+        }
     }
     if (c.pif) { if (n > 1) d += PIb[(size_t)i * PIFS + PIF_D + pi_tri(r, r)]; }
     else {
@@ -1470,6 +1489,7 @@
     const int sel = a.use_cur ? __builtin_amdgcn_readfirstlane(a.w.lm[b].cur) : 0;
     c.buf = sel; c.x = a.x + (size_t)b * n * 15;
     c.PL = sel ? a.w.PL[1] : a.w.PL[0]; c.PI = sel ? a.w.PI[1] : a.w.PI[0]; c.PW = sel ? a.w.PW[1] : a.w.PW[0]; c.PG = sel ? a.w.PG[1] : a.w.PG[0];
+    c.PP = sel ? a.w.PP[1] : a.w.PP[0]; c.CS = sel ? a.w.CS[1] : a.w.CS[0];
     STAMPM(5000);
     for (int e = lane; e < 256; e += 64) { T.CD[e] = 0.0; T.W[e] = 0.0; }
     if (lane < 16) T.Cg[lane] = 0.0;
diff --git a/2dliw-slam_amd/csrc/k_lm_quad.hip b/2dliw-slam_amd/csrc/k_lm_quad.hip
--- a/2dliw-slam_amd/csrc/k_lm_quad.hip
+++ b/2dliw-slam_amd/csrc/k_lm_quad.hip
@@ -89,8 +89,10 @@
     return R <= j ? cR + j : cj + R;
 }
 
+template <bool FOLD>
 __global__ __launch_bounds__(64, 1) void k_lm_step_quad(StepArgs a) {
     __shared__ double S[QTOT];
+    constexpr int SW = FOLD ? PPS : PWS, SG = FOLD ? 0 : PGS;
     const int lane = threadIdx.x & 63, j = lane & 15, w = lane >> 4;
     const int n = a.n;
     const bool track = a.mode == LIW_MODE_TRACK;
@@ -236,7 +238,7 @@
     const double* const PG0 = a.w.PG[0];
     const unsigned oPL = (unsigned)b * (unsigned)(n * LPC) + (cur ? (unsigned)(a.w.PL[1] - a.w.PL[0]) : 0u);
     const unsigned oPI = (unsigned)b * (unsigned)(n * PIFS) + (cur ? (unsigned)(a.w.PI[1] - a.w.PI[0]) : 0u);
-    const unsigned oPW = (unsigned)b * (unsigned)((n - 1) * PWS) + (cur ? (unsigned)(a.w.PW[1] - a.w.PW[0]) : 0u);
+    const unsigned oPW = (unsigned)b * (unsigned)(FOLD ? n * PPS : (n - 1) * PWS) + (cur ? (unsigned)(a.w.PW[1] - a.w.PW[0]) : 0u);
     const unsigned oPG = (unsigned)b * (unsigned)(n * PGS) + (cur ? (unsigned)(a.w.PG[1] - a.w.PG[0]) : 0u);
     const unsigned oWS = (unsigned)b * (unsigned)(n * SOLVE_WS);
     double* const WS = a.w.solve_ws;
@@ -258,9 +260,13 @@
                 const int j6 = l6 ? jc : 0;
                 vbb[u] = PL0[oPL + (unsigned)(i * LPC + (cbb >= 0 ? cbb & 63 : 0))];
                 vbb[u] = cbb >= 0 ? vbb[u] : 0.0;
-                vjj[u] = n > 1 ? PW0[oPW + (unsigned)(max(i - 1, 0) * PWS + PW_JJ(j6, j6))] : 0.0;
-                vii[u] = n > 1 ? PW0[oPW + (unsigned)(min(i, n - 2) * PWS + PW_II(j6, j6))] : 0.0;
-                vg[u] = PG0[oPG + (unsigned)(i * PGS + PG_H(j6, j6))];
+                if constexpr (FOLD) {
+                    vjj[u] = PW0[oPW + (unsigned)(i * PPS + PP_H(j6, j6))]; vii[u] = 0.0; vg[u] = 0.0;
+                } else {
+                    vjj[u] = n > 1 ? PW0[oPW + (unsigned)(max(i - 1, 0) * PWS + PW_JJ(j6, j6))] : 0.0;
+                    vii[u] = n > 1 ? PW0[oPW + (unsigned)(min(i, n - 2) * PWS + PW_II(j6, j6))] : 0.0;
+                    vg[u] = PG0[oPG + (unsigned)(i * PGS + PG_H(j6, j6))];
+                }
                 vi[u] = PI0[oPI + (unsigned)(i * PIFS + PIF_D + pi_tri(jc, jc))];
             }
 #pragma unroll
@@ -271,9 +277,12 @@
                 if (l6) {
                     dd += vbb[u];
                     if (i == 0) for (int f = 0; f < n; ++f) { const double va = PL0[oPL + (unsigned)(f * LPC + (caa >= 0 ? caa & 63 : 0))]; dd += caa >= 0 ? va : 0.0; }
-                    if (i >= 1) dd += vjj[u];
-                    if (i <= n - 2) dd += vii[u];
-                    dd += vg[u];
+                    if constexpr (FOLD) dd += vjj[u];
+                    else {
+                        if (i >= 1) dd += vjj[u];
+                        if (i <= n - 2) dd += vii[u];
+                        dd += vg[u];
+                    }
                 }
                 if (n > 1) dd += vi[u];
                 if (prior_row && i == n - 2) dd += sp;
@@ -283,7 +292,7 @@
     }
     const double sc0 = l6 ? LMD[oSC + (unsigned)jc] : 0.0;
 
-    constexpr int S_IMU = 0, S_PL = 4 * PIFS, S_PW = S_PL + 4 * LPC, S_PG = S_PW + 4 * PWS, S_TR = S_PG + 4 * PGS + QPAD;
+    constexpr int S_IMU = 0, S_PL = 4 * PIFS, S_PW = S_PL + 4 * LPC, S_PG = S_PW + 4 * SW, S_TR = S_PG + 4 * SG + QPAD;
     constexpr int S_ZERO = S_TR + QTR, S_TAB = S_ZERO + QZB;
     static_assert(S_TAB + QTAB <= QTOT && 8 * QTOT < 65536, "LDS layout");
     const unsigned rPI[4] = {(unsigned)__builtin_amdgcn_readlane(oPI, 0), (unsigned)__builtin_amdgcn_readlane(oPI, 16), (unsigned)__builtin_amdgcn_readlane(oPI, 32), (unsigned)__builtin_amdgcn_readlane(oPI, 48)};
@@ -314,16 +323,16 @@
             });
         }
         {
-            const unsigned fl = (unsigned)(f * LPC), fw = (unsigned)((k >= 0 ? k : 0) * PWS), fg = (unsigned)(f * PGS);
-            constexpr int NPC = (4 * (LPC + PWS + PGS) + 127) / 128;
-            static_assert(NPC * 128 - 4 * (LPC + PWS + PGS) <= QPAD && LPC % 2 == 0 && PWS % 2 == 0 && PGS % 2 == 0, "stream pieces: pad, 16-byte slots");
+            const unsigned fl = (unsigned)(f * LPC), fw = FOLD ? (unsigned)(f * PPS) : (unsigned)((k >= 0 ? k : 0) * PWS), fg = (unsigned)(f * PGS);
+            constexpr int NPC = (4 * (LPC + SW + SG) + 127) / 128, NGR = FOLD ? 8 : 12;
+            static_assert(NPC * 128 - 4 * (LPC + SW + SG) <= QPAD && LPC % 2 == 0 && SW % 2 == 0 && SG % 2 == 0, "stream pieces: pad, 16-byte slots");
             sfor<0, NPC>([&](auto P) {
                 constexpr int q0 = KI(P) * 128;
                 unsigned off = 0;
-                sfor<0, 12>([&](auto G) {
+                sfor<0, NGR>([&](auto G) {
                     constexpr int g = KI(G);
-                    constexpr int st = g < 4 ? g * LPC : g < 8 ? 4 * LPC + (g - 4) * PWS : 4 * (LPC + PWS) + (g - 8) * PGS;
-                    constexpr int en = g == 11 ? (1 << 20) : st + (g < 4 ? LPC : g < 8 ? PWS : PGS);
+                    constexpr int st = g < 4 ? g * LPC : g < 8 ? 4 * LPC + (g - 4) * SW : 4 * (LPC + SW) + (g - 8) * SG;
+                    constexpr int en = g == NGR - 1 ? (1 << 20) : st + (g < 4 ? LPC : g < 8 ? SW : SG);
                     if constexpr (st < q0 + 128 && en > q0) {
                         const unsigned v = (g < 4 ? rPLw[g & 3] + fl : g < 8 ? rPW[g & 3] + fw : rPGw[g & 3] + fg) + (unsigned)(lane2 - (st - q0));
                         if constexpr (st <= q0) off = v; else off = lane2 >= st - q0 ? v : off;
@@ -340,7 +349,7 @@
     {
         const int jt = j < 15 ? j : 0, cjt = 14 * jt - (jt * (jt - 1)) / 2, j6t = j < 6 ? j : 0;
         const bool t6 = j < 6, t15 = j == 15, tm = j < 15;
-        const int oL = S_PL + w * LPC, oW_ = S_PW + w * PWS, oG = S_PG + w * PGS, oI = S_IMU + w * PIFS;
+        const int oL = S_PL + w * LPC, oW_ = S_PW + w * SW, oG = S_PG + w * SG, oI = S_IMU + w * PIFS;
         auto put = [&](int k, bool on, int idx) { TAB[k * 64 + lane] = (unsigned short)(8 * (on ? idx : S_ZERO)); };
         const int role = t15 ? 6 : j6t;
         auto put_laser = [&](int k, bool on, int code) { put(k, on && code >= 0, oL + (code & 63)); };
@@ -348,13 +357,18 @@
         sfor<0, 6>([&](auto R) {
             constexpr int r = KI(R);
             put_laser(K_A + r, t6 || t15, quad_code<0, r>(track, role));
-            put(K_B + r, t6 || t15, oW_ + (t15 ? PW_G(6 + r) : PW_JJ(r, j6t)));
-            put(K_C + r, t6 || t15, oG + (t15 ? PG_G(r) : PG_H(r, j6t)));
+            if constexpr (FOLD) {
+                put(K_B + r, t6 || t15, oW_ + (t15 ? PP_G + r : PP_H(r, j6t)));
+                put(K_C + r, false, 0);
+            } else {
+                put(K_B + r, t6 || t15, oW_ + (t15 ? PW_G(6 + r) : PW_JJ(r, j6t)));
+                put(K_C + r, t6 || t15, oG + (t15 ? PG_G(r) : PG_H(r, j6t)));
+            }
             put_laser(K_HA + r, t6 || t15, quad_code<1, r>(track, role));
-            put(K_CW + r, t6 || t15, oW_ + (t15 ? PW_G(r) : PW_II(r, j6t)));
+            put(K_CW + r, !FOLD && (t6 || t15), oW_ + (t15 ? PW_G(r) : PW_II(r, j6t)));
             put_laser(K_RL + r, t6, quad_code<2, r>(track, role));
         });
-        put(K_GSH, t6, oW_ + PW_G(j6t));
+        put(K_GSH, !FOLD && t6, oW_ + PW_G(j6t));
         sfor<0, 15>([&](auto R) {
             constexpr int r = KI(R);
             put(K_D + r, tm, oI + PIF_D + tri_rc<r>(jt, cjt));
@@ -404,14 +418,15 @@
             constexpr int NT = K_D - K_A;
             unsigned of[NT + 15], ofR[6];
             auto tab_at = [&](int k) { return (unsigned)*reinterpret_cast<const unsigned short*>(reinterpret_cast<const char*>(TAB) + k * 128 + lane_tab); };
-            sfor<0, NT>([&](auto Q) { constexpr int q = KI(Q); of[q] = tab_at(K_A + q); });
+            constexpr auto rd_used = [](int q) { return !(FOLD && q >= K_C - K_A && q < K_C - K_A + 6); };
+            sfor<0, NT>([&](auto Q) { constexpr int q = KI(Q); if constexpr (rd_used(q)) of[q] = tab_at(K_A + q); });
             sfor<0, 6>([&](auto Q) { constexpr int q = KI(Q); ofR[q] = tab_at(K_RL + q); });
             if (n > 1) sfor<0, 15>([&](auto Q) { constexpr int q = KI(Q); of[NT + q] = tab_at(K_D + q); });
             const char* const Sb = reinterpret_cast<const char*>(S);
             const int w8 = (lane >> 4) * 8;
             const char* const bOV = Sb + (l15 ? 8 * (S_IMU + PIF_GJ) : 8 * (S_IMU + PIF_IJ) + jc * 120) + w8 * PIFS;
             const char* const bGI = Sb + (l15 ? 8 * (S_IMU + PIF_GI) + w8 * PIFS : 8 * S_ZERO);
-            const char* const bOW = Sb + (l6 ? 8 * (S_PW + PW_IJ(0, 0)) + w8 * PWS + j6 * 48 : 8 * S_ZERO);
+            const char* const bOW = Sb + (l6 ? 8 * (S_PW + (FOLD ? PP_IJ : PW_IJ(0, 0))) + w8 * SW + j6 * 48 : 8 * S_ZERO);
             double gi[15];
             if (n > 1) {
                 sfor<0, 15>([&](auto R) { constexpr int r = KI(R); o[r] = *reinterpret_cast<const double*>(bOV + 8 * r); gi[r] = *reinterpret_cast<const double*>(bGI + 8 * r); });
@@ -421,14 +436,18 @@
             sfor<0, 6>([&](auto R) { constexpr int r = KI(R); oW[r] = *reinterpret_cast<const double*>(bOW + 8 * r); });
             asm volatile("" ::: "memory");
             double pb[NT];
-            sfor<0, NT>([&](auto Q) { constexpr int q = KI(Q); pb[q] = *reinterpret_cast<const double*>(Sb + of[q]); });
+            sfor<0, NT>([&](auto Q) { constexpr int q = KI(Q); if constexpr (rd_used(q)) pb[q] = *reinterpret_cast<const double*>(Sb + of[q]); });
             sfor<0, 6>([&](auto R) { constexpr int r = KI(R); rL[r] = *reinterpret_cast<const double*>(Sb + ofR[r]); });
             if (n > 1) sfor<0, 15>([&](auto Q) { constexpr int q = KI(Q); d[q] = *reinterpret_cast<const double*>(Sb + of[NT + q]); });
             asm volatile("" ::: "memory");
             pb[K_A + 0] = flip_sign(pb[K_A + 0], sgA0); pb[K_A + 1] = flip_sign(pb[K_A + 1], sgA0);
             pb[K_A + 3] = flip_sign(pb[K_A + 3], sgA3); pb[K_A + 4] = flip_sign(pb[K_A + 4], sgA3); pb[K_A + 5] = flip_sign(pb[K_A + 5], sgA3);
             rL[0] = flip_sign(rL[0], sgR0); rL[1] = flip_sign(rL[1], sgR0);
-            sfor<0, 6>([&](auto R) { constexpr int r = KI(R); tS[r] = pb[K_A + r] + bits_and(pb[K_B + r], mh) + pb[K_C + r]; });
+            sfor<0, 6>([&](auto R) {
+                constexpr int r = KI(R);
+                if constexpr (FOLD) tS[r] = pb[K_A + r] + pb[K_B + r];
+                else tS[r] = pb[K_A + r] + bits_and(pb[K_B + r], mh) + pb[K_C + r];
+            });
             if (!track) {
                 sfor<0, 6>([&](auto R) { constexpr int r = KI(R); hA[r] += pb[K_HA + r]; });
                 if (i == 0) sfor<0, 6>([&](auto R) { tS[KI(R)] += hA[KI(R)]; });
@@ -524,7 +543,9 @@
             });
         }
         QSTAMP(5);
-        if (hasm) {
+        if constexpr (FOLD) {
+            sfor<0, 15>([&](auto R) { cd[KI(R)] = 0.0; });
+        } else if (hasm) {
             dpp_fence();
             double cw[6];
             sfor<0, 6>([&](auto R) { constexpr int r = KI(R); cw[r] = RD(KC<K_CW + r>{}); });
@@ -768,7 +789,7 @@
     return a.n >= 1 && (a.mode == LIW_MODE_INIT || (a.mode == LIW_MODE_TRACK && a.n >= 2)) && span(a.w.PL[0], a.w.PL[1], (unsigned long long)a.n * LPC) && a.w.pi_frame && a.w.pl_compact &&
            a.w.PL[0] >= a.w.PW[0] && span(a.w.PW[0], a.w.PL[1], (unsigned long long)a.n * LPC) &&
            a.w.CS[0] && a.w.CS[1] && span(a.w.PI[0], a.w.PI[1], (unsigned long long)a.n * PIFS) &&
-           span(a.w.PW[0], a.w.PW[1], (unsigned long long)nm * PWS) && span(a.w.PG[0], a.w.PG[1], (unsigned long long)a.n * PGS) &&
+           span(a.w.PW[0], a.w.PW[1], a.w.pose_fold ? (unsigned long long)a.n * PPS : (unsigned long long)nm * PWS) && span(a.w.PG[0], a.w.PG[1], (unsigned long long)a.n * PGS) &&
            a.w.PG[0] >= a.w.PW[0] && span(a.w.PW[0], a.w.PG[1], (unsigned long long)a.n * PGS) &&
            (unsigned long long)a.B * (sizeof(LmState) / 8) <= lim && (unsigned long long)a.B * a.n * SOLVE_WS <= lim;
 }
@@ -778,7 +799,8 @@
     if (out) (void)hipMemcpyFromSymbol(out, HIP_SYMBOL(g_qclk), sizeof(long long) * 64);
 }
 void launch_lm_step_quad(const StepArgs& a, hipStream_t s) {
-    hipLaunchKernelGGL(k_lm_step_quad, dim3((a.B + 3) / 4), dim3(64), 0, s, a);
-}
-
-}
+    if (a.w.pose_fold) hipLaunchKernelGGL(k_lm_step_quad<true>, dim3((a.B + 3) / 4), dim3(64), 0, s, a);
+    else hipLaunchKernelGGL(k_lm_step_quad<false>, dim3((a.B + 3) / 4), dim3(64), 0, s, a);
+}
+
+}
diff --git a/2dliw-slam_amd/csrc/liw_capi.hip b/2dliw-slam_amd/csrc/liw_capi.hip
--- a/2dliw-slam_amd/csrc/liw_capi.hip
+++ b/2dliw-slam_amd/csrc/liw_capi.hip
@@ -221,7 +221,7 @@
     const int nm = n > 1 ? n - 1 : 1;
     const int lps = laser_stride(pi_frame_format(B) ? 1 : 0);
     for (int k = 0; k < 2; ++k) { f.PI[k] = o; o = al256(o + sizeof(double) * (size_t)B * pi_doubles_per_window(n)); }
-    for (int k = 0; k < 2; ++k) { f.PW[k] = o; o = al256(o + sizeof(double) * (size_t)B * nm * PWS); }
+    for (int k = 0; k < 2; ++k) { f.PW[k] = o; o = al256(o + sizeof(double) * (size_t)B * (pi_frame_format(B) ? pw_doubles_per_window(n) : (size_t)nm * PWS)); }
     for (int k = 0; k < 2; ++k) { f.PL[k] = o; o = al256(o + sizeof(double) * (size_t)B * n * lps); }
     for (int k = 0; k < 2; ++k) { f.PG[k] = o; o = al256(o + sizeof(double) * (size_t)B * n * PGS); }
     f.x_cand = o; o = al256(o + sizeof(double) * (size_t)B * n * 15);
@@ -256,6 +256,8 @@
     v.active = (int*)(base + f.active);
     v.pi_frame = pi_frame_format(B) ? 1 : 0;
     v.pl_compact = v.pi_frame;
+    v.pose_fold = pose_fold_format(B, n) ? 1 : 0;
+    for (int k = 0; k < 2; ++k) v.PP[k] = v.PW[k];
     for (int k = 0; k < 2; ++k) v.CS[k] = (double*)(base + f.CS[k]);
     v.imu_pk = (double*)(base + f.imu_pk);
     v.imu_pk_bad = (int*)(base + f.imu_pk_bad);
@@ -321,6 +323,8 @@
     A.candidate = candidate;
     A.pi_frame = v.pi_frame;
     A.pl_compact = v.pl_compact;
+    A.pose_fold = v.pose_fold;
+    for (int k = 0; k < 2; ++k) A.PP[k] = v.PP[k];
     for (int k = 0; k < 2; ++k) A.CS[k] = v.pi_frame ? v.CS[k] : nullptr;
     if (packed && b->n > 1 && b->eval_small) { A.imu_pk = v.imu_pk; A.imu_pk_bad = v.imu_pk_bad; }
     if (packed) A.laser_hz = v.imu_pk_bad + 1;
diff --git a/2dliw-slam_amd/csrc/liw_kernels.hpp b/2dliw-slam_amd/csrc/liw_kernels.hpp
--- a/2dliw-slam_amd/csrc/liw_kernels.hpp
+++ b/2dliw-slam_amd/csrc/liw_kernels.hpp
@@ -55,6 +55,13 @@
 __host__ __device__ constexpr int PG_H(int r, int c) { return tri_sym<7>(r, c); }
 __host__ __device__ constexpr int PG_G(int r) { return tri_sym<7>(r, 6); }
 constexpr int PG_C = 27;
+constexpr int PPS = 64, PP_D = 0, PP_G = 21, PP_IJ = 28;
+__host__ __device__ constexpr int PP_H(int r, int c) { return PP_D + tri_sym<6>(r, c); }
+inline bool pose_fold_format(int B, int n) { return n > 1 && pi_frame_format(B) && getenv("LIW_NO_POSE_FOLD") == nullptr; }
+__host__ __device__ inline size_t pw_doubles_per_window(int n) {
+    const size_t a = (size_t)(n > 1 ? n - 1 : 1) * PWS, b = (size_t)n * PPS;
+    return a > b ? a : b;
+}
 constexpr int FTF = 32;
 
 struct LmState {
@@ -86,6 +93,8 @@
     int* active;
     int pi_frame;
     int pl_compact;
+    int pose_fold;
+    double* PP[2];
     double* CS[2];
     double* imu_pk;
     int* imu_pk_bad;
@@ -118,6 +127,8 @@
     int* active;
     int pi_frame;
     int pl_compact;
+    int pose_fold;
+    double* PP[2];
     double* CS[2];
     const double* imu_pk;
     const int* imu_pk_bad;
```
